# raulmur/ORB_SLAM2

Measured on NVIDIA H100. Metric: stereo frames/sec (ORB extract L+R + ComputeStereoMatches, KITTI-shaped 1242x375 @2000 kpts), higher is better.
Workload: dtype u8

## Files before the change

### include/borb.h

```cpp
#ifndef BORB_H
#define BORB_H

#include <stddef.h>
#include <stdint.h>

#if defined(__GNUC__)
#define BORB_API __attribute__((visibility("default")))
#else
#define BORB_API
#endif

#ifdef __cplusplus
extern "C" {
#endif

#define BORB_VERSION 2
#define BORB_MAX_LEVELS 16
#define BORB_MAX_DIM 4095

typedef enum borb_status {
    BORB_OK = 0,
    BORB_ERR_INVALID_ARG = 1,
    BORB_ERR_NO_DEVICE = 2,
    BORB_ERR_CUDA = 3,
    BORB_ERR_UNSUPPORTED = 4,
    BORB_ERR_CAPACITY = 5,
    BORB_ERR_STATE = 6
} borb_status;

typedef struct borb_keypoint {
    float x, y;
    float size;
    float angle;
    float response;
    int32_t octave;
    int32_t class_id;
} borb_keypoint;

typedef struct borb_extractor_cfg {
    int32_t n_features;
    float scale_factor;
    int32_t n_levels;
    int32_t ini_th_fast;
    int32_t min_th_fast;
} borb_extractor_cfg;

typedef struct borb_extractor borb_extractor;

BORB_API const char* borb_last_error(void);
BORB_API const char* borb_status_str(borb_status s);
BORB_API int borb_version(void);
BORB_API borb_status borb_device_count(int* n);

BORB_API borb_status borb_host_alloc(void** p, size_t bytes);
BORB_API borb_status borb_host_free(void* p);

BORB_API borb_status borb_extractor_create(const borb_extractor_cfg* cfg, int device, borb_extractor** out);
BORB_API borb_status borb_extractor_destroy(borb_extractor* e);
BORB_API borb_status borb_extractor_tables(const borb_extractor* e, float* scale, float* inv_scale, float* sigma2,
                                  float* inv_sigma2, int32_t* features_per_level);
BORB_API borb_status borb_extractor_capacity(const borb_extractor* e, int width, int height, int* cap);
BORB_API borb_status borb_extractor_reserve(borb_extractor* e, int width, int height, int max_images);

BORB_API borb_status borb_extract(borb_extractor* e, const uint8_t* gray, int width, int height, int stride,
                         borb_keypoint* kps, uint8_t* desc, int cap, int* n_out);

BORB_API borb_status borb_extract_batch(borb_extractor* e, const uint8_t* const* gray, int n_images, int width, int height,
                               int stride, borb_keypoint* kps, uint8_t* desc, int cap, int* n_out);

BORB_API borb_status borb_extract_batch_enqueue(borb_extractor* e, const uint8_t* const* gray, int n_images, int width,
                                       int height, int stride, borb_keypoint* kps, uint8_t* desc, int cap, int* n_out);
BORB_API borb_status borb_sync(borb_extractor* e);

BORB_API borb_status borb_extract_batch_device(borb_extractor* e, const uint8_t* d_gray, int n_images, int width, int height,
                                      size_t pitch, size_t image_stride, borb_keypoint* kps, uint8_t* desc, int cap,
                                      int* n_out);

BORB_API borb_status borb_extractor_set_input_format(borb_extractor* e, int channels, int rgb_order);

BORB_API borb_status borb_extractor_set_rectify_maps(borb_extractor* e, int which, const float* map_x, const float* map_y, int src_w,
                                                     int src_h, int dst_w, int dst_h);

BORB_API borb_status borb_extractor_pyramid(borb_extractor* e, int image, int level, uint8_t* dst, int* w, int* h);

BORB_API borb_status borb_stereo_match(borb_extractor* e, int n_pairs, const int* left_idx, const int* right_idx, float bf,
                              float b, float* u_right, float* depth, int cap);

BORB_API borb_status borb_stereo_match2(borb_extractor* left, borb_extractor* right, float bf, float b, float* u_right,
                               float* depth, int cap);

BORB_API borb_status borb_stereo_frames(borb_extractor* e, const uint8_t* const* left, const uint8_t* const* right, int n_pairs,
                               int width, int height, int stride, float bf, float b, borb_keypoint* kps_left,
                               uint8_t* desc_left, int* n_left, borb_keypoint* kps_right, uint8_t* desc_right,
                               int* n_right, float* u_right, float* depth, int cap);
BORB_API borb_status borb_stereo_frames_enqueue(borb_extractor* e, const uint8_t* const* left, const uint8_t* const* right,
                                       int n_pairs, int width, int height, int stride, float bf, float b,
                                       borb_keypoint* kps_left, uint8_t* desc_left, int* n_left,
                                       borb_keypoint* kps_right, uint8_t* desc_right, int* n_right, float* u_right,
                                       float* depth, int cap);
BORB_API borb_status borb_stereo_frames_device_enqueue(borb_extractor* e, const uint8_t* d_gray, int n_pairs, int width,
                                              int height, size_t pitch, size_t image_stride, float bf, float b,
                                              int* n_left, int* n_right, float* u_right, float* depth, int cap);
BORB_API borb_status borb_stereo_frames_device(borb_extractor* e, const uint8_t* d_gray, int n_pairs, int width, int height,
                                      size_t pitch, size_t image_stride, float bf, float b, int* n_left, int* n_right,
                                      float* u_right, float* depth, int cap);
BORB_API borb_status borb_stereo_frames_results(borb_extractor* e, int n_pairs, borb_keypoint* kps_left, uint8_t* desc_left,
                                                int* n_left, borb_keypoint* kps_right, uint8_t* desc_right, int* n_right,
                                                float* u_right, float* depth, int cap);

typedef struct borb_matcher borb_matcher;
#define BORB_MATCH_MAX_FEATURES 8192
BORB_API borb_status borb_matcher_create(int device, borb_matcher** out);
BORB_API borb_status borb_matcher_destroy(borb_matcher* m);

typedef struct borb_frame borb_frame;
typedef struct borb_frame_view {
    int32_t n;
    const borb_keypoint* keys_un;
    const uint8_t* desc;
    const float* u_right;
    const uint8_t* occupied;
    float min_x, min_y, max_x, max_y;
    int32_t n_levels;
    const float* scale_factors;
    const borb_frame* resident;
} borb_frame_view;

BORB_API borb_status borb_frame_create(borb_matcher* m, const borb_frame_view* view, borb_frame** out);
BORB_API borb_status borb_frame_destroy(borb_frame* f);

typedef struct borb_camera {
    float fx, fy, cx, cy;
    float k1, k2, p1, p2, k3;
    float bf;
} borb_camera;

BORB_API borb_status borb_frames_from_extractor(borb_matcher* m, borb_extractor* e, const int32_t* images, int n_frames,
                                                const int32_t* n_keys, const borb_camera* cam, int mode, const void* const* depth,
                                                int depth_type, float depth_factor, int depth_stride_bytes, borb_keypoint* keys_un,
                                                float* u_right, float* depth_out, int cap, float* bounds4, borb_frame** frames);
BORB_API borb_status borb_frame_info(const borb_frame* f, int32_t* n, int32_t* n_levels, int32_t* has_u_right);

typedef struct borb_mappoint_view {
    int32_t n;
    const float* proj_x;
    const float* proj_y;
    const float* proj_xr;
    const int32_t* level;
    const float* view_cos;
    const uint8_t* desc;
    const uint8_t* valid;
    const uint8_t* has_obs;
} borb_mappoint_view;

BORB_API borb_status borb_search_by_projection(borb_matcher* m, const borb_frame_view* frame, const borb_mappoint_view* mps,
                                               float th, float nnratio, int32_t* match_feat, int32_t* n_matches);
BORB_API borb_status borb_search_by_projection_batch(borb_matcher* m, const borb_frame_view* frames, const borb_mappoint_view* points,
                                                     int n_jobs, float th, float nnratio, int32_t* const* match_feat, int32_t* n_matches);

typedef struct borb_lastframe_view {
    int32_t n;
    const borb_keypoint* keys_un;
    const float* world_pos;
    const uint8_t* desc;
    const uint8_t* valid;
    const uint8_t* has_obs;
} borb_lastframe_view;

BORB_API borb_status borb_search_by_projection_last(borb_matcher* m, const borb_frame_view* cur, const borb_lastframe_view* last,
                                                    const float* Tcw, float fx, float fy, float cx, float cy, float bf, float th,
                                                    int forward, int backward, int check_orientation, int32_t* state_cur,
                                                    int32_t* n_matches);

typedef struct borb_worldpoints_view {
    int32_t n;
    const float* world_pos;
    const uint8_t* desc;
    const float* max_distance;
    const float* min_distance;
    const float* normal;
    const float* angle;
    const uint8_t* valid;
} borb_worldpoints_view;

BORB_API borb_status borb_search_by_projection_kf(borb_matcher* m, const borb_frame_view* cur, const borb_worldpoints_view* pts,
                                                  const float* Tcw, const float* Ow, float fx, float fy, float cx, float cy,
                                                  float log_scale_factor, float th, int orb_dist, int check_orientation,
                                                  int32_t* state_cur, int32_t* n_matches);

BORB_API borb_status borb_search_by_projection_sim3(borb_matcher* m, const borb_frame_view* kf, const borb_worldpoints_view* pts,
                                                    const float* Tcw, const float* Ow, float fx, float fy, float cx, float cy,
                                                    float log_scale_factor, int th, int32_t* state_kf, int32_t* n_matches);

BORB_API borb_status borb_fuse(borb_matcher* m, const borb_frame_view* kf, const float* inv_level_sigma2,
                               const borb_worldpoints_view* pts, const float* Tcw, const float* Ow, float fx, float fy, float cx,
                               float cy, float bf, float log_scale_factor, float th, int scw_variant, int32_t* best_idx,
                               int32_t* n_found);

BORB_API borb_status borb_search_by_sim3(borb_matcher* m, const borb_frame_view* kf1, const borb_frame_view* kf2,
                                         const borb_worldpoints_view* pts1, const borb_worldpoints_view* pts2, const float* T1w,
                                         const float* T2w, const float* S12, const float* S21, float fx, float fy, float cx, float cy,
                                         float log_scale_factor1, float log_scale_factor2, float th, int32_t* match12,
                                         int32_t* n_found);

BORB_API borb_status borb_search_local_points(borb_matcher* m, const borb_frame_view* frame, const borb_worldpoints_view* pts,
                                              const uint8_t* has_obs, const float* Tcw, const float* Ow, float fx, float fy, float cx,
                                              float cy, float mbf, float viewing_cos_limit, float log_scale_factor, float th,
                                              float nnratio, uint8_t* in_view, float* proj_x, float* proj_y, float* proj_xr,
                                              int32_t* level, float* view_cos, int32_t* match_feat, int32_t* n_matches);

typedef struct borb_local_points_job {
    borb_frame_view frame;
    borb_worldpoints_view pts;
    const uint8_t* has_obs;
    float Tcw[12];
    float Ow[3];
    float fx, fy, cx, cy, mbf;
    float log_scale_factor;
    float th;
    uint8_t* in_view;
    float* proj_x;
    float* proj_y;
    float* proj_xr;
    int32_t* level;
    float* view_cos;
    int32_t* match_feat;
} borb_local_points_job;
BORB_API borb_status borb_search_local_points_batch(borb_matcher* m, const borb_local_points_job* jobs, int n_jobs, float viewing_cos_limit,
                                                    float nnratio, int32_t* n_matches);

typedef struct borb_last_frame_job {
    borb_frame_view cur;
    borb_lastframe_view last;
    float Tcw[12];
    float fx, fy, cx, cy, bf;
    float th;
    int32_t forward, backward;
    int32_t* state_cur;
} borb_last_frame_job;
BORB_API borb_status borb_search_by_projection_last_batch(borb_matcher* m, const borb_last_frame_job* jobs, int n_jobs, int check_orientation,
                                                          int32_t* n_matches);

BORB_API borb_status borb_search_for_initialization(borb_matcher* m, const borb_frame_view* f1, const borb_frame_view* f2,
                                                    float* prev_matched, int window_size, float nnratio, int check_orientation,
                                                    int32_t* matches12, int32_t* n_matches);

BORB_API borb_status borb_distinctive_descriptors(borb_matcher* m, const uint8_t* desc, const int32_t* offsets, int n_points,
                                                  int32_t* best_idx);

typedef struct borb_featvec_view {
    int32_t n_nodes;
    const uint32_t* node_id;
    const int32_t* start;
    const uint32_t* feat_idx;
} borb_featvec_view;

typedef struct borb_keyframe_view {
    int32_t n;
    const borb_keypoint* keys_un;
    const uint8_t* desc;
    const uint8_t* has_mp;
    const float* u_right;
    borb_featvec_view fv;
    int32_t n_levels;
    const float* scale_factors;
    const float* level_sigma2;
} borb_keyframe_view;

BORB_API borb_status borb_search_by_bow(borb_matcher* m, const borb_keyframe_view* kfs, int n_kf, const borb_keyframe_view* frame,
                                        float nnratio, int check_orientation, int32_t* match, int32_t* n_matches);
BORB_API borb_status borb_search_by_bow_kf(borb_matcher* m, const borb_keyframe_view* kf1, const borb_keyframe_view* kf2,
                                           float nnratio, int check_orientation, int32_t* match12, int32_t* n_matches);

typedef struct borb_bow_job {
    const borb_frame* frame;
    borb_keyframe_view kf;
    const borb_frame* kf_frame;
    int32_t* match;
} borb_bow_job;
BORB_API borb_status borb_search_by_bow_batch(borb_matcher* m, const borb_bow_job* jobs, int n_jobs, float nnratio,
                                              int check_orientation, int32_t* n_matches);
BORB_API borb_status borb_search_for_triangulation(borb_matcher* m, const borb_keyframe_view* kf1, const borb_keyframe_view* kf2,
                                                   const float* F12, float ex, float ey, int only_stereo, int check_orientation,
                                                   int32_t* pairs, int cap, int32_t* n_pairs);

typedef struct borb_kfdb borb_kfdb;
BORB_API borb_status borb_kfdb_create(int device, borb_kfdb** out);
BORB_API borb_status borb_kfdb_destroy(borb_kfdb* db);
BORB_API borb_status borb_kfdb_clear(borb_kfdb* db);
BORB_API borb_status borb_kfdb_add(borb_kfdb* db, const borb_keyframe_view* kf, const uint32_t* bow_word, const double* bow_value,
                                   int n_bow, int32_t* slot_out);
BORB_API borb_status borb_kfdb_erase(borb_kfdb* db, int32_t slot);
BORB_API borb_status borb_kfdb_set_has_mp(borb_kfdb* db, int32_t slot, const uint8_t* has_mp);
BORB_API borb_status borb_kfdb_size(const borb_kfdb* db, int32_t* n_slots, uint64_t* device_bytes);
BORB_API borb_status borb_kfdb_query(borb_matcher* m, borb_kfdb* db, const uint32_t* bow_word, const double* bow_value, int n_bow,
                                     int32_t* common_words, float* score, uint32_t* first_word, int cap, int32_t* n_slots);
BORB_API borb_status borb_search_by_bow_db(borb_matcher* m, borb_kfdb* db, const int32_t* slots, int n_kf,
                                           const borb_keyframe_view* frame, float nnratio, int check_orientation, int32_t* match,
                                           int32_t* n_matches);

BORB_API borb_status borb_search_by_bow_db_pairs(borb_matcher* m, borb_kfdb* db, const int32_t* slots, int n_kf,
                                                 const borb_keyframe_view* frame, float nnratio, int check_orientation,
                                                 int32_t* n_matches, int32_t* pair_offset, uint32_t* pairs, int pairs_cap,
                                                 int32_t* n_pairs_total);

typedef struct borb_voc borb_voc;
BORB_API borb_status borb_voc_create(const int32_t* parent, const uint8_t* is_leaf, const uint8_t* desc, const double* weight,
                                     int n_nodes, int k, int L, int device, borb_voc** out);
BORB_API borb_status borb_voc_load_text(const char* path, int device, borb_voc** out);
BORB_API borb_status borb_voc_destroy(borb_voc* v);
BORB_API borb_status borb_voc_blob(const borb_voc* v, void** d_blob, size_t* bytes);
BORB_API borb_status borb_voc_from_blob(void* d_blob, size_t bytes, int device, borb_voc** out);
BORB_API borb_status borb_nccl_unique_id(uint8_t* id128);
BORB_API borb_status borb_nccl_comm_create(const uint8_t* id128, int world_size, int rank, int device, void** nccl_comm);
BORB_API borb_status borb_nccl_comm_destroy(void* nccl_comm);
BORB_API borb_status borb_voc_broadcast(borb_voc* root_voc, void* nccl_comm, int root, int rank, int device, borb_voc** out);

BORB_API borb_status borb_bow_transform(borb_voc* v, const uint8_t* desc, int n, int levelsup, int32_t* word, double* weight,
                                        int32_t* node);

BORB_API borb_status borb_compute_bow(borb_voc* v, const uint8_t* desc, int n, int levelsup, uint32_t* bow_word, double* bow_value,
                                      int32_t* n_bow, uint32_t* fv_node, int32_t* fv_start, uint32_t* fv_idx, int32_t* n_nodes);

BORB_API borb_status borb_frames_compute_bow(borb_matcher* m, borb_voc* v, borb_frame* const* frames, int n_frames, int levelsup,
                                             uint32_t* const* bow_word, double* const* bow_value, int32_t* n_bow,
                                             uint32_t* const* fv_node, int32_t* const* fv_start, uint32_t* const* fv_idx,
                                             int32_t* n_nodes);

BORB_API borb_status borb_matcher_set_timing(borb_matcher* m, int enable);
BORB_API borb_status borb_matcher_last_kernel_ms(borb_matcher* m, float* ms);
BORB_API borb_status borb_matcher_launch_count(const borb_matcher* m, uint64_t* n);
BORB_API borb_status borb_debug_candidates(borb_extractor* e, int image, int level, int32_t* xys, int cap, int* n_out);
BORB_API borb_status borb_debug_selected(borb_extractor* e, int image, int level, int32_t* xys, int cap, int* n_out);
BORB_API borb_status borb_debug_blurred(borb_extractor* e, int image, int level, uint8_t* dst, int* w, int* h);
BORB_API borb_status borb_debug_set_fast_mode(borb_extractor* e, int mode);
BORB_API borb_status borb_debug_brief_slots(uint32_t* dst, int cap, int* n_bins);
BORB_API borb_status borb_debug_set_bow_csa(int mode);
BORB_API borb_status borb_debug_set_bow_item_target(int target);
BORB_API borb_status borb_launch_count(const borb_extractor* e, uint64_t* n);
BORB_API borb_status borb_stage_times(borb_extractor* e, float* ms8);
BORB_API borb_status borb_set_timing(borb_extractor* e, int enable);
BORB_API borb_status borb_stage_times_total(borb_extractor* e, double* ms8, uint64_t* steps);
BORB_API borb_status borb_extractor_stream(borb_extractor* e, void** stream);

#ifdef __cplusplus
}
#endif
#endif
```

### orb_slam2_b200/_lib.py

```python
from __future__ import annotations

import ctypes as C
import os

import numpy as np

HERE = os.path.dirname(os.path.abspath(__file__))
LIB_PATH = os.path.join(HERE, "libborb.so")

KP_DTYPE = np.dtype([("x", "<f4"), ("y", "<f4"), ("size", "<f4"), ("angle", "<f4"), ("response", "<f4"),
                     ("octave", "<i4"), ("class_id", "<i4")])

BORB_OK = 0
STATUS_NAMES = {0: "BORB_OK", 1: "BORB_ERR_INVALID_ARG", 2: "BORB_ERR_NO_DEVICE", 3: "BORB_ERR_CUDA",
                4: "BORB_ERR_UNSUPPORTED", 5: "BORB_ERR_CAPACITY", 6: "BORB_ERR_STATE"}


class BorbError(RuntimeError):
    def __init__(self, status: int, where: str, detail: str):
        self.status = status
        super().__init__(f"{where}: {STATUS_NAMES.get(status, status)}: {detail}")


class ExtractorCfg(C.Structure):
    _fields_ = [("n_features", C.c_int32), ("scale_factor", C.c_float), ("n_levels", C.c_int32),
                ("ini_th_fast", C.c_int32), ("min_th_fast", C.c_int32)]


u8p = C.POINTER(C.c_uint8)
f32p = C.POINTER(C.c_float)
i32p = C.POINTER(C.c_int32)
vp = C.c_void_p

_SIGNATURES = {
    "borb_last_error": (C.c_char_p, []),
    "borb_status_str": (C.c_char_p, [C.c_int]),
    "borb_version": (C.c_int, []),
    "borb_device_count": (C.c_int, [i32p]),
    "borb_host_alloc": (C.c_int, [C.POINTER(vp), C.c_size_t]),
    "borb_host_free": (C.c_int, [vp]),
    "borb_extractor_create": (C.c_int, [C.POINTER(ExtractorCfg), C.c_int, C.POINTER(vp)]),
    "borb_extractor_destroy": (C.c_int, [vp]),
    "borb_extractor_tables": (C.c_int, [vp, f32p, f32p, f32p, f32p, i32p]),
    "borb_extractor_capacity": (C.c_int, [vp, C.c_int, C.c_int, i32p]),
    "borb_extractor_reserve": (C.c_int, [vp, C.c_int, C.c_int, C.c_int]),
    "borb_extract": (C.c_int, [vp, vp, C.c_int, C.c_int, C.c_int, vp, vp, C.c_int, i32p]),
    "borb_extract_batch": (C.c_int, [vp, C.POINTER(vp), C.c_int, C.c_int, C.c_int, C.c_int, vp, vp, C.c_int, vp]),
    "borb_extract_batch_enqueue": (C.c_int, [vp, C.POINTER(vp), C.c_int, C.c_int, C.c_int, C.c_int, vp, vp, C.c_int, vp]),
    "borb_sync": (C.c_int, [vp]),
    "borb_extract_batch_device": (C.c_int, [vp, vp, C.c_int, C.c_int, C.c_int, C.c_size_t, C.c_size_t, vp, vp, C.c_int, vp]),
    "borb_extractor_pyramid": (C.c_int, [vp, C.c_int, C.c_int, vp, i32p, i32p]),
    "borb_stereo_match": (C.c_int, [vp, C.c_int, vp, vp, C.c_float, C.c_float, vp, vp, C.c_int]),
    "borb_stereo_match2": (C.c_int, [vp, vp, C.c_float, C.c_float, vp, vp, C.c_int]),
    "borb_stereo_frames": (C.c_int, [vp, C.POINTER(vp), C.POINTER(vp), C.c_int, C.c_int, C.c_int, C.c_int, C.c_float,
                                     C.c_float, vp, vp, vp, vp, vp, vp, vp, vp, C.c_int]),
    "borb_stereo_frames_enqueue": (C.c_int, [vp, C.POINTER(vp), C.POINTER(vp), C.c_int, C.c_int, C.c_int, C.c_int,
                                             C.c_float, C.c_float, vp, vp, vp, vp, vp, vp, vp, vp, C.c_int]),
    "borb_stereo_frames_device": (C.c_int, [vp, vp, C.c_int, C.c_int, C.c_int, C.c_size_t, C.c_size_t, C.c_float,
                                            C.c_float, vp, vp, vp, vp, C.c_int]),
    "borb_stereo_frames_device_enqueue": (C.c_int, [vp, vp, C.c_int, C.c_int, C.c_int, C.c_size_t, C.c_size_t, C.c_float,
                                                    C.c_float, vp, vp, vp, vp, C.c_int]),
    "borb_stereo_frames_results": (C.c_int, [vp, C.c_int, vp, vp, vp, vp, vp, vp, vp, vp, C.c_int]),
    "borb_stage_times_total": (C.c_int, [vp, C.POINTER(C.c_double), C.POINTER(C.c_uint64)]),
    "borb_extractor_stream": (C.c_int, [vp, C.POINTER(vp)]),
    "borb_matcher_create": (C.c_int, [C.c_int, C.POINTER(vp)]),
    "borb_extractor_set_input_format": (C.c_int, [vp, C.c_int, C.c_int]),
    "borb_extractor_set_rectify_maps": (C.c_int, [vp, C.c_int, vp, vp, C.c_int, C.c_int, C.c_int, C.c_int]),
    "borb_matcher_destroy": (C.c_int, [vp]),
    "borb_frame_create": (C.c_int, [vp, vp, C.POINTER(vp)]),
    "borb_frame_destroy": (C.c_int, [vp]),
    "borb_frames_from_extractor": (C.c_int, [vp, vp, vp, C.c_int, vp, vp, C.c_int, vp, C.c_int, C.c_float, C.c_int, vp, vp, vp, C.c_int, vp, vp]),
    "borb_frame_info": (C.c_int, [vp, i32p, i32p, i32p]),
    "borb_search_by_projection": (C.c_int, [vp, vp, vp, C.c_float, C.c_float, vp, i32p]),
    "borb_search_by_projection_batch": (C.c_int, [vp, vp, vp, C.c_int, C.c_float, C.c_float, vp, vp]),
    "borb_search_by_projection_last": (C.c_int, [vp, vp, vp, vp, C.c_float, C.c_float, C.c_float, C.c_float, C.c_float, C.c_float,
                                                 C.c_int, C.c_int, C.c_int, vp, i32p]),
    "borb_search_by_projection_kf": (C.c_int, [vp, vp, vp, vp, vp, C.c_float, C.c_float, C.c_float, C.c_float, C.c_float, C.c_float,
                                               C.c_int, C.c_int, vp, i32p]),
    "borb_search_by_projection_sim3": (C.c_int, [vp, vp, vp, vp, vp, C.c_float, C.c_float, C.c_float, C.c_float, C.c_float, C.c_int,
                                                 vp, i32p]),
    "borb_search_for_initialization": (C.c_int, [vp, vp, vp, vp, C.c_int, C.c_float, C.c_int, vp, i32p]),
    "borb_distinctive_descriptors": (C.c_int, [vp, vp, vp, C.c_int, vp]),
    "borb_kfdb_create": (C.c_int, [C.c_int, C.POINTER(vp)]),
    "borb_kfdb_destroy": (C.c_int, [vp]),
    "borb_kfdb_clear": (C.c_int, [vp]),
    "borb_kfdb_add": (C.c_int, [vp, vp, vp, vp, C.c_int, i32p]),
    "borb_kfdb_erase": (C.c_int, [vp, C.c_int32]),
    "borb_kfdb_set_has_mp": (C.c_int, [vp, C.c_int32, vp]),
    "borb_kfdb_size": (C.c_int, [vp, i32p, C.POINTER(C.c_uint64)]),
    "borb_kfdb_query": (C.c_int, [vp, vp, vp, vp, C.c_int, vp, vp, vp, C.c_int, i32p]),
    "borb_search_by_bow_db": (C.c_int, [vp, vp, vp, C.c_int, vp, C.c_float, C.c_int, vp, vp]),
    "borb_search_by_bow_db_pairs": (C.c_int, [vp, vp, vp, C.c_int, vp, C.c_float, C.c_int, vp, vp, vp, C.c_int, i32p]),
    "borb_search_local_points": (C.c_int, [vp, vp, vp, vp, vp, vp] + [C.c_float] * 9 + [vp] * 7 + [i32p]),
    "borb_search_local_points_batch": (C.c_int, [vp, vp, C.c_int, C.c_float, C.c_float, vp]),
    "borb_search_by_projection_last_batch": (C.c_int, [vp, vp, C.c_int, C.c_int, vp]),
    "borb_fuse": (C.c_int, [vp, vp, vp, vp, vp, vp, C.c_float, C.c_float, C.c_float, C.c_float, C.c_float, C.c_float, C.c_float, C.c_int,
                            vp, i32p]),
    "borb_search_by_sim3": (C.c_int, [vp, vp, vp, vp, vp, vp, vp, vp, vp, C.c_float, C.c_float, C.c_float, C.c_float, C.c_float, C.c_float,
                                      C.c_float, vp, i32p]),
    "borb_search_by_bow": (C.c_int, [vp, vp, C.c_int, vp, C.c_float, C.c_int, vp, vp]),
    "borb_search_by_bow_kf": (C.c_int, [vp, vp, vp, C.c_float, C.c_int, vp, i32p]),
    "borb_search_by_bow_batch": (C.c_int, [vp, vp, C.c_int, C.c_float, C.c_int, vp]),
    "borb_frames_compute_bow": (C.c_int, [vp, vp, vp, C.c_int, C.c_int, vp, vp, vp, vp, vp, vp, vp]),
    "borb_search_for_triangulation": (C.c_int, [vp, vp, vp, vp, C.c_float, C.c_float, C.c_int, C.c_int, vp, C.c_int, i32p]),
    "borb_voc_create": (C.c_int, [vp, vp, vp, vp, C.c_int, C.c_int, C.c_int, C.c_int, C.POINTER(vp)]),
    "borb_voc_load_text": (C.c_int, [C.c_char_p, C.c_int, C.POINTER(vp)]),
    "borb_voc_destroy": (C.c_int, [vp]),
    "borb_voc_blob": (C.c_int, [vp, C.POINTER(vp), C.POINTER(C.c_size_t)]),
    "borb_voc_from_blob": (C.c_int, [vp, C.c_size_t, C.c_int, C.POINTER(vp)]),
    "borb_bow_transform": (C.c_int, [vp, vp, C.c_int, C.c_int, vp, vp, vp]),
    "borb_debug_candidates": (C.c_int, [vp, C.c_int, C.c_int, vp, C.c_int, i32p]),
    "borb_debug_selected": (C.c_int, [vp, C.c_int, C.c_int, vp, C.c_int, i32p]),
    "borb_debug_blurred": (C.c_int, [vp, C.c_int, C.c_int, vp, i32p, i32p]),
    "borb_nccl_unique_id": (C.c_int, [vp]),
    "borb_nccl_comm_create": (C.c_int, [vp, C.c_int, C.c_int, C.c_int, C.POINTER(vp)]),
    "borb_nccl_comm_destroy": (C.c_int, [vp]),
    "borb_voc_broadcast": (C.c_int, [vp, vp, C.c_int, C.c_int, C.c_int, C.POINTER(vp)]),
    "borb_compute_bow": (C.c_int, [vp, vp, C.c_int, C.c_int, vp, vp, i32p, vp, vp, vp, i32p]),
    "borb_matcher_set_timing": (C.c_int, [vp, C.c_int]),
    "borb_matcher_last_kernel_ms": (C.c_int, [vp, f32p]),
    "borb_matcher_launch_count": (C.c_int, [vp, C.POINTER(C.c_uint64)]),
    "borb_debug_set_bow_csa": (C.c_int, [C.c_int]),
    "borb_debug_set_bow_item_target": (C.c_int, [C.c_int]),
    "borb_debug_set_fast_mode": (C.c_int, [vp, C.c_int]),
    "borb_debug_brief_slots": (C.c_int, [vp, C.c_int, i32p]),
    "borb_launch_count": (C.c_int, [vp, C.POINTER(C.c_uint64)]),
    "borb_stage_times": (C.c_int, [vp, f32p]),
    "borb_set_timing": (C.c_int, [vp, C.c_int]),
}

_lib = None


def exported_names():
    return sorted(_SIGNATURES)


def load() -> C.CDLL:
    global _lib
    if _lib is not None:
        return _lib
    if not os.path.exists(LIB_PATH):
        raise ImportError(f"{LIB_PATH} is missing: build it with `python -c 'import __graft_entry__ as g; g.build()'` "
                          "(orb_slam2_b200 has no CPU fallback)")
    lib = C.CDLL(LIB_PATH)
    for name, (res, args) in _SIGNATURES.items():
        fn = getattr(lib, name)
        fn.restype = res
        fn.argtypes = args
    _lib = lib
    return lib


def check(status: int, where: str) -> None:
    if status != BORB_OK:
        detail = load().borb_last_error()
        raise BorbError(status, where, detail.decode() if detail else "")


def device_count() -> int:
    n = C.c_int32(0)
    st = load().borb_device_count(C.byref(n))
    return n.value if st == BORB_OK else 0


def ptr(a: np.ndarray):
    return a.ctypes.data_as(vp) if a is not None else None
```

### orb_slam2_b200/csrc/borb_host.cu

```cuda
#include <cmath>
#include <cstdarg>
#include <cstdio>
#include <algorithm>
#include <cstdlib>
#include <cstring>

#include "borb_internal.h"

namespace borb {

static thread_local std::string tl_error;
void set_error(const char* fmt, ...) {
    char buf[512];
    va_list ap;
    va_start(ap, fmt);
    vsnprintf(buf, sizeof(buf), fmt, ap);
    va_end(ap);
    tl_error = buf;
}

bool allow_max_smem(const void* func) {
    static std::mutex mu;
    static std::vector<std::pair<const void*, int>> done;
    int dev = 0;
    if (cudaGetDevice(&dev) != cudaSuccess) return false;
    std::lock_guard<std::mutex> lk(mu);
    for (auto& d : done)
        if (d.first == func && d.second == dev) return true;
    cudaFuncAttributes fa;
    int optin = 0;
    cudaError_t e = cudaFuncGetAttributes(&fa, func);
    if (e == cudaSuccess) e = cudaDeviceGetAttribute(&optin, cudaDevAttrMaxSharedMemoryPerBlockOptin, dev);
    if (e == cudaSuccess) e = cudaFuncSetAttribute(func, cudaFuncAttributeMaxDynamicSharedMemorySize, optin - (int)fa.sharedSizeBytes);
    if (e != cudaSuccess) { set_error("raising the shared-memory limit failed: %s", cudaGetErrorString(e)); cudaGetLastError(); return false; }
    done.push_back({func, dev});
    return true;
}

namespace {

inline int cv_round_f(float v) { return (int)lrintf(v); }
inline int align_up(int v, int a) { return (v + a - 1) / a * a; }

void init_tables(borb_extractor* e) {
    const int L = e->cfg.n_levels;
    const double sf = (double)e->cfg.scale_factor;
    e->scale.assign(L, 1.f); e->sigma2.assign(L, 1.f); e->inv_scale.assign(L, 1.f); e->inv_sigma2.assign(L, 1.f);
    for (int i = 1; i < L; i++) {
        e->scale[i] = (float)((double)e->scale[i - 1] * sf);
        e->sigma2[i] = e->scale[i] * e->scale[i];
    }
    for (int i = 0; i < L; i++) { e->inv_scale[i] = 1.0f / e->scale[i]; e->inv_sigma2[i] = 1.0f / e->sigma2[i]; }
    e->per_level.assign(L, 0);
    const float factor = (float)(1.0 / sf);
    float want = (float)e->cfg.n_features * (1.f - factor) / (1.f - (float)std::pow((double)factor, (double)L));
    int sum = 0;
    for (int l = 0; l < L - 1; l++) {
        e->per_level[l] = cv_round_f(want);
        sum += e->per_level[l];
        want *= factor;
    }
    e->per_level[L - 1] = e->cfg.n_features - sum > 0 ? e->cfg.n_features - sum : 0;
    const int vmax = (int)std::floor(HALF_PATCH * std::sqrt(2.f) / 2 + 1);
    const int vmin = (int)std::ceil(HALF_PATCH * std::sqrt(2.f) / 2);
    for (int v = 0; v < 16; v++) e->umax[v] = 0;
    for (int v = 0; v <= vmax; ++v) e->umax[v] = (int)lrint(std::sqrt((double)HALF_PATCH * HALF_PATCH - (double)v * v));
    for (int v = HALF_PATCH, v0 = 0; v >= vmin; --v) {
        while (e->umax[v0] == e->umax[v0 + 1]) ++v0;
        e->umax[v] = v0;
        ++v0;
    }
}

void resize_table(int src, int dst, bool clamp_edges, int extra, std::vector<int16_t>& out) {
    const double inv = (double)dst / src, scale = 1. / inv;
    const size_t first = out.size();
    for (int d = 0; d < dst; d++) {
        float f = (float)((d + 0.5) * scale - 0.5);
        int s = (int)std::floor(f);
        f -= s;
        if (clamp_edges) {
            if (s < 0) { f = 0; s = 0; }
            if (s >= src - 1) { f = 0; s = src - 1; }
        }
        out.push_back((int16_t)s);
        out.push_back((int16_t)cv_round_f((1.f - f) * 2048.f));
        out.push_back((int16_t)cv_round_f(f * 2048.f));
        out.push_back(0);
    }
    for (int k = 0; k < extra; k++) {
        int r = 2 * dst - 2 - (dst + k);
        if (r < 0) r = 0;
        for (int j = 0; j < 4; j++) out.push_back(out[first + (size_t)r * 4 + j]);
    }
    if (((out.size() - first) / 4) & 1) for (int j = 0; j < 4; j++) out.push_back(0);
}

bool resize_window_table(const std::vector<int16_t>& tabs, size_t xtab_first, int n_entries, std::vector<int16_t>& out) {
    bool ok = true;
    for (int gq = 0; gq < n_entries; gq += 4) {
        int lo = 1 << 30, hi = 0;
        for (int i = 0; i < 4; i++) {
            const int ofs = tabs[xtab_first + (size_t)(gq + i) * 4];
            lo = std::min(lo, ofs); hi = std::max(hi, ofs);
        }
        const int base = lo & ~3;
        if (hi + 1 - base > 11) ok = false;
        for (int i = 0; i < 4; i++) {
            const int16_t* e = &tabs[xtab_first + (size_t)(gq + i) * 4];
            const int pos = e[0] - base;
            int s1 = 0, s2 = 0x10;
            if (pos <= 6) s1 = pos | ((pos + 1) << 4);
            else if (pos == 7) { s1 = 7; s2 = 0x40; }
            else { const int q = (pos - 8) + 4; s2 = q | ((q + 1) << 4); }
            out.push_back(e[1]);
            out.push_back(e[2]);
            out.push_back((int16_t)base);
            out.push_back((int16_t)((s1 | (s2 << 8)) & 0x7FFF));
        }
    }
    return ok;
}

const int8_t kPattern[1024] = {
#include "orb_pattern.inc"
};

borb_status build_geometry(borb_extractor* e, int w, int h, std::vector<int16_t>& tabs) {
    Geometry& g = e->geom;
    std::memset(&g, 0, sizeof(g));
    const int L = e->cfg.n_levels;
    g.nlevels = L; g.w = w; g.h = h;
    g.fast_mode = e->fast_mode;
    g.ini_th = e->cfg.ini_th_fast < 0 ? 0 : (e->cfg.ini_th_fast > 255 ? 255 : e->cfg.ini_th_fast);
    g.min_th = e->cfg.min_th_fast < 0 ? 0 : (e->cfg.min_th_fast > 255 ? 255 : e->cfg.min_th_fast);
    for (int i = 0; i < 16; i++) g.umax[i] = e->umax[i];
    unsigned pyr_off = 0, cand_off = 0;
    int blk = 0, sel_off = 0, btile = 0;
    tabs.clear();
    for (int l = 0; l < L; l++) {
        LevelGeom& v = g.lv[l];
        v.w = cv_round_f((float)w * e->inv_scale[l]);
        v.h = cv_round_f((float)h * e->inv_scale[l]);
        const float width = (float)(v.w - 2 * MIN_BORDER), height = (float)(v.h - 2 * MIN_BORDER);
        v.nCols = (int)(width / 30.f);
        v.nRows = (int)(height / 30.f);
        if (v.nCols < 1 || v.nRows < 1) {
            set_error("level %d is %dx%d: too small for the 30-px FAST cell grid (reference divides by zero)", l, v.w, v.h);
            return BORB_ERR_UNSUPPORTED;
        }
        v.wCell = (int)std::ceil(width / v.nCols);
        v.hCell = (int)std::ceil(height / v.nRows);
        v.pitch = align_up(v.w + 8, 128);
        v.pyr_off = pyr_off;
        pyr_off += (unsigned)v.pitch * v.h;
        v.cellsPerBlk = FAST_TILE_W / v.wCell > 0 ? FAST_TILE_W / v.wCell : 1;
        v.rowsPerBlk = fast_rows_per_blk(v.nRows, v.hCell);
        v.blkCols = (v.nCols + v.cellsPerBlk - 1) / v.cellsPerBlk;
        v.blkBase = blk;
        blk += v.blkCols * ((v.nRows + v.rowsPerBlk - 1) / v.rowsPerBlk);
        v.cand_off = cand_off;
        v.cand_cap = v.nCols * v.nRows * ((v.wCell + 1) / 2) * ((v.hCell + 1) / 2);
        cand_off += (unsigned)align_up(v.cand_cap, 32);
        v.quota = e->per_level[l];
        v.nIni = (int)std::round(width / height);
        if (v.nIni < 1) { set_error("level %d aspect ratio gives zero quadtree roots (reference divides by zero)", l); return BORB_ERR_UNSUPPORTED; }
        v.hX = width / v.nIni;
        v.node_cap = (v.quota > 4 * v.nIni ? v.quota : 4 * v.nIni) + 3;
        v.node_cap = align_up(v.node_cap + 1, 4);
        v.sel_off = sel_off;
        sel_off += v.node_cap;
        v.scale = e->scale[l];
        v.inv_scale = e->inv_scale[l];
        v.patch_size = (float)(int)(PATCH * e->scale[l]);
        g.blur_base[l] = btile;
        btile += ((v.w + BLUR_TILE_W - 1) / BLUR_TILE_W) * ((v.h + BLUR_TILE_H - 1) / BLUR_TILE_H);
        if (l > 0) {
            const int wpad = (v.w + 8 + 3) & ~3;
            v.xtab_off = (unsigned)(tabs.size() / 4);
            resize_table(g.lv[l - 1].w, v.w, true, wpad - v.w, tabs);
            v.ytab_off = (unsigned)(tabs.size() / 4);
            resize_table(g.lv[l - 1].h, v.h, false, 0, tabs);
            v.xwin_off = (unsigned)(tabs.size() / 4);
            std::vector<int16_t> win;
            v.x_windowed = resize_window_table(tabs, (size_t)v.xtab_off * 4, wpad, win) ? 1 : 0;
            tabs.insert(tabs.end(), win.begin(), win.end());
        }
        if (quadtree_smem_bytes(v.node_cap) > 200 * 1024) {
            set_error("per-level quota %d exceeds the quadtree kernel's shared-memory envelope", v.quota);
            return BORB_ERR_UNSUPPORTED;
        }
    }
    g.blur_base[L] = btile;
    g.blur_tiles = btile;
    g.fast_blocks = blk;
    g.pyr_image_stride = (unsigned)align_up((int)pyr_off, g.lv[0].pitch);
    g.cand_image_stride = cand_off;
    g.sel_image_stride = sel_off;
    if (sel_off >= 65536) { set_error("keypoint capacity %d exceeds 65535", sel_off); return BORB_ERR_UNSUPPORTED; }
    return BORB_OK;
}

void free_workspace(Workspace& ws) {
    cudaFree(ws.pyr); cudaFree(ws.blur); cudaFree(ws.cand); cudaFree(ws.cand_cnt); cudaFree(ws.pnode); cudaFree(ws.sel);
    cudaFree(ws.sel_cnt); cudaFree(ws.kps); cudaFree(ws.desc); cudaFree(ws.nkp); cudaFree(ws.u_right); cudaFree(ws.depth);
    cudaFree(ws.sad); cudaFree(ws.tabs); cudaFree(ws.brief_slots); cudaFree(ws.pair_idx); cudaFree(ws.st_bins); cudaFree(ws.st_recs); cudaFree(ws.stage);
    free(ws.fast_tmaps); cudaFree(ws.fast_tiles);
    ws = Workspace();
}

borb_status ensure(borb_extractor* e, int w, int h, int n_images) {
    if (w < 1 || h < 1 || w > BORB_MAX_DIM || h > BORB_MAX_DIM) { set_error("image size %dx%d outside [1,%d]", w, h, BORB_MAX_DIM); return BORB_ERR_UNSUPPORTED; }
    BORB_CUDA(cudaSetDevice(e->device));
    const bool same_shape = e->have_geom && e->geom.w == w && e->geom.h == h;
    if (same_shape && e->ws.max_images >= n_images) return BORB_OK;
    BORB_CUDA(cudaStreamSynchronize(e->stream));
    std::vector<int16_t> tabs;
    e->have_geom = false;
    e->last_n_images = 0;
    e->last_stereo_pairs = 0;
    borb_status st = build_geometry(e, w, h, tabs);
    if (st != BORB_OK) return st;
    size_t n = (size_t)(n_images > 2 ? n_images : 2);
    if (same_shape && (size_t)e->ws.max_images > n) n = (size_t)e->ws.max_images;
    free_workspace(e->ws);
    if (e->h_counts) { cudaFreeHost(e->h_counts); e->h_counts = nullptr; }
    e->pair_cache.clear();
    const Geometry& g = e->geom;
    Workspace& ws = e->ws;
    BORB_CUDA(cudaMalloc(&ws.pyr, n * g.pyr_image_stride + 256));
    BORB_CUDA(cudaMalloc(&ws.blur, n * g.pyr_image_stride + 256));
    BORB_CUDA(cudaMalloc(&ws.cand, n * g.cand_image_stride * sizeof(uint32_t)));
    BORB_CUDA(cudaMalloc(&ws.pnode, n * g.cand_image_stride * sizeof(int)));
    BORB_CUDA(cudaMalloc(&ws.cand_cnt, n * g.nlevels * sizeof(int)));
    BORB_CUDA(cudaMalloc(&ws.sel, n * g.sel_image_stride * sizeof(uint32_t)));
    BORB_CUDA(cudaMalloc(&ws.sel_cnt, n * g.nlevels * sizeof(int)));
    BORB_CUDA(cudaMalloc(&ws.kps, n * g.sel_image_stride * sizeof(borb_keypoint)));
    BORB_CUDA(cudaMalloc(&ws.desc, n * g.sel_image_stride * 32));
    BORB_CUDA(cudaMalloc(&ws.nkp, n * sizeof(int)));
    BORB_CUDA(cudaMalloc(&ws.u_right, n * g.sel_image_stride * sizeof(float)));
    BORB_CUDA(cudaMalloc(&ws.depth, n * g.sel_image_stride * sizeof(float)));
    BORB_CUDA(cudaMalloc(&ws.sad, n * g.sel_image_stride * sizeof(int)));
    BORB_CUDA(cudaMalloc(&ws.pair_idx, n * 2 * sizeof(int)));
    BORB_CUDA(cudaMalloc(&ws.st_bins, n * stereo_bins_bytes_per_pair()));
    BORB_CUDA(cudaMalloc(&ws.st_recs, n * (size_t)stereo_rec_stride(g) * stereo_rec_bytes()));
    BORB_CUDA(cudaMalloc(&ws.tabs, (tabs.size() + 4) * sizeof(int16_t)));
    BORB_CUDA(cudaMemcpy(ws.tabs, tabs.data(), tabs.size() * sizeof(int16_t), cudaMemcpyHostToDevice));
    const std::vector<uint32_t>& slots = brief_slot_table();
    BORB_CUDA(cudaMalloc(&ws.brief_slots, slots.size() * sizeof(uint32_t)));
    BORB_CUDA(cudaMemcpy(ws.brief_slots, slots.data(), slots.size() * sizeof(uint32_t), cudaMemcpyHostToDevice));
    BORB_CUDA(cudaMemset(ws.nkp, 0, n * sizeof(int)));
    BORB_CUDA(cudaMallocHost(&e->h_counts, n * 2 * sizeof(int)));
    ws.max_images = (int)n;
    ws.fast_tmaps = malloc(fast_tmaps_bytes());
    if ((st = build_fast_tmaps(g, ws, ws.fast_tmaps)) != BORB_OK) return st;
    if ((st = build_fast_tiles(g, ws)) != BORB_OK) return st;
    e->have_geom = true;
    return BORB_OK;
}

void drain_timing(borb_extractor* e);
void begin_step(borb_extractor* e) {
    if (!e->timing) return;
    if (e->ev.empty()) {
        e->ev.resize((size_t)borb_extractor::EV_RING * 9);
        for (auto& x : e->ev) cudaEventCreate(&x);
    }
    if (e->ev_pending >= borb_extractor::EV_RING) {
        cudaStreamSynchronize(e->stream);
        drain_timing(e);
    }
    e->ev_slot = (e->ev_slot + 1) % borb_extractor::EV_RING;
    e->ev_mask[e->ev_slot] = 0;
    e->ev_pending++;
}
void mark(borb_extractor* e, int i) {
    if (!e->timing || e->ev.empty()) return;
    cudaEventRecord(e->ev[(size_t)e->ev_slot * 9 + i], e->stream);
    e->ev_mask[e->ev_slot] |= 1u << i;
}
void drain_timing(borb_extractor* e) {
    const int R = borb_extractor::EV_RING;
    for (int k = e->ev_pending - 1; k >= 0; k--) {
        const int slot = ((e->ev_slot - k) % R + R) % R;
        const unsigned m = e->ev_mask[slot];
        for (int i = 0; i < 8; i++) {
            float ms = 0.f;
            if (m & (1u << i)) {
                int j = i + 1;
                while (j < 9 && !(m & (1u << j))) j++;
                if (j < 9 && cudaEventElapsedTime(&ms, e->ev[(size_t)slot * 9 + i], e->ev[(size_t)slot * 9 + j]) != cudaSuccess) { ms = 0.f; cudaGetLastError(); }
            }
            e->stage_ms[i] = ms;
            e->stage_sum_ms[i] += ms;
        }
        e->stage_steps++;
    }
    e->ev_pending = 0;
}

borb_status enqueue_extract(borb_extractor* e, int n) {
    const Geometry& g = e->geom;
    Workspace& ws = e->ws;
    cudaStream_t s = e->stream;
    BORB_CUDA(cudaMemsetAsync(ws.cand_cnt, 0, (size_t)n * g.nlevels * sizeof(int), s));
    mark(e, 1);
    e->launches += launch_pyramid(g, ws, n, s);
    mark(e, 2);
    e->launches += launch_fast(g, ws, n, s);
    mark(e, 3);
    e->launches += launch_quadtree(g, ws, n, s);
    mark(e, 4);
    e->launches += launch_blur(g, ws, n, s);
    mark(e, 5);
    e->launches += launch_describe(g, ws, n, s);
    mark(e, 6);
    BORB_CUDA(cudaGetLastError());
    e->last_n_images = n;
    e->last_stereo_pairs = 0;
    return BORB_OK;
}

borb_status rectified_size(borb_extractor* e, int w, int h, int* gw, int* gh) {
    if (!e->d_map[0][0]) return BORB_OK;
    if (w != e->map_src_w || h != e->map_src_h) {
        set_error("rectification maps were built for %dx%d raw frames, got %dx%d", e->map_src_w, e->map_src_h, w, h);
        return BORB_ERR_INVALID_ARG;
    }
    *gw = e->map_dst_w; *gh = e->map_dst_h;
    return BORB_OK;
}

borb_status upload_slots(borb_extractor* e, const uint8_t* const* slots, int n, int w, int h, int stride, bool stereo_pairs = false) {
    const Geometry& g = e->geom;
    const int ch = e->in_channels;
    if (stride < w * ch) { set_error("stride %d smaller than a row of %d %d-channel pixels", stride, w, ch); return BORB_ERR_INVALID_ARG; }
    const size_t img_bytes = (size_t)stride * h;
    bool contiguous = n > 1 || ch > 1 || e->d_map[0][0] != nullptr;
    for (int k = 0; k < n; k++) {
        if (!slots[k]) { set_error("image %d is NULL", k); return BORB_ERR_INVALID_ARG; }
        if (slots[k] != slots[0] + (size_t)k * img_bytes) contiguous = false;
    }
    auto need_stage = [&](size_t need) -> borb_status {
        if (e->ws.stage_bytes < need) {
            BORB_CUDA(cudaStreamSynchronize(e->stream));
            cudaFree(e->ws.stage);
            e->ws.stage = nullptr; e->ws.stage_bytes = 0;
            BORB_CUDA(cudaMalloc(&e->ws.stage, need));
            e->ws.stage_bytes = need;
        }
        return BORB_OK;
    };
    if (e->d_map[0][0]) {
        if (ch != 1) { set_error("rectification maps apply to CV_8UC1 frames"); return BORB_ERR_UNSUPPORTED; }
        const size_t src_img = contiguous ? img_bytes : (size_t)w * h;
        const int src_stride = contiguous ? stride : w;
        borb_status st = need_stage(src_img * n);
        if (st != BORB_OK) return st;
        if (contiguous) BORB_CUDA(cudaMemcpyAsync(e->ws.stage, slots[0], src_img * n, cudaMemcpyHostToDevice, e->stream));
        else
            for (int k = 0; k < n; k++)
                BORB_CUDA(cudaMemcpy2DAsync(e->ws.stage + (size_t)k * src_img, w, slots[k], stride, w, h, cudaMemcpyHostToDevice, e->stream));
        e->launches += launch_repack_remap(g, e->ws, e->ws.stage, src_stride, src_img, w, h, e->d_map[0][0], e->d_map[0][1],
                                           stereo_pairs ? e->d_map[1][0] : nullptr, stereo_pairs ? e->d_map[1][1] : nullptr, n, e->stream);
        return BORB_OK;
    }
    if (contiguous) {
        const size_t need = img_bytes * n;
        borb_status st = need_stage(need);
        if (st != BORB_OK) return st;
        BORB_CUDA(cudaMemcpyAsync(e->ws.stage, slots[0], need, cudaMemcpyHostToDevice, e->stream));
        if (ch == 1) e->launches += launch_repack(g, e->ws, e->ws.stage, stride, img_bytes, n, e->stream);
        else e->launches += launch_repack_color(g, e->ws, e->ws.stage, stride, img_bytes, ch, e->in_rgb, n, e->stream);
        return BORB_OK;
    }
    if (ch > 1) {
        const size_t row = (size_t)w * ch;
        borb_status st = need_stage(row * h * n);
        if (st != BORB_OK) return st;
        for (int k = 0; k < n; k++)
            BORB_CUDA(cudaMemcpy2DAsync(e->ws.stage + (size_t)k * row * h, row, slots[k], stride, row, h, cudaMemcpyHostToDevice, e->stream));
        e->launches += launch_repack_color(g, e->ws, e->ws.stage, (int)row, row * h, ch, e->in_rgb, n, e->stream);
        return BORB_OK;
    }
    for (int k = 0; k < n; k++) {
        uint8_t* dst = e->ws.pyr + (size_t)k * g.pyr_image_stride + g.lv[0].pyr_off;
        BORB_CUDA(cudaMemcpy2DAsync(dst, g.lv[0].pitch, slots[k], stride, w, h, cudaMemcpyHostToDevice, e->stream));
    }
    return BORB_OK;
}

borb_status upload_device(borb_extractor* e, const uint8_t* d_gray, int n, int w, int h, size_t pitch, size_t image_stride) {
    const Geometry& g = e->geom;
    cudaMemcpy3DParms p = {};
    p.srcPtr = make_cudaPitchedPtr((void*)d_gray, pitch, w, image_stride / pitch);
    p.dstPtr = make_cudaPitchedPtr(e->ws.pyr + g.lv[0].pyr_off, g.lv[0].pitch, w, g.pyr_image_stride / g.lv[0].pitch);
    if (image_stride % pitch == 0 && g.pyr_image_stride % g.lv[0].pitch == 0) {
        p.extent = make_cudaExtent(w, h, n);
        p.kind = cudaMemcpyDeviceToDevice;
        BORB_CUDA(cudaMemcpy3DAsync(&p, e->stream));
    } else {
        for (int i = 0; i < n; i++)
            BORB_CUDA(cudaMemcpy2DAsync(e->ws.pyr + (size_t)i * g.pyr_image_stride + g.lv[0].pyr_off, g.lv[0].pitch,
                                        d_gray + (size_t)i * image_stride, pitch, w, h, cudaMemcpyDeviceToDevice, e->stream));
    }
    return BORB_OK;
}

borb_status download_kps(borb_extractor* e, int first, int count, int step, borb_keypoint* kps, uint8_t* desc, int cap, int* n_out) {
    const Geometry& g = e->geom;
    const int m = cap < g.sel_image_stride ? cap : g.sel_image_stride;
    cudaStream_t s = e->stream;
    if (kps && m > 0)
        BORB_CUDA(cudaMemcpy2DAsync(kps, (size_t)cap * sizeof(borb_keypoint), e->ws.kps + (size_t)first * g.sel_image_stride,
                                    (size_t)step * g.sel_image_stride * sizeof(borb_keypoint), (size_t)m * sizeof(borb_keypoint),
                                    count, cudaMemcpyDeviceToHost, s));
    if (desc && m > 0)
        BORB_CUDA(cudaMemcpy2DAsync(desc, (size_t)cap * 32, e->ws.desc + (size_t)first * g.sel_image_stride * 32,
                                    (size_t)step * g.sel_image_stride * 32, (size_t)m * 32, count, cudaMemcpyDeviceToHost, s));
    if (n_out)
        BORB_CUDA(cudaMemcpy2DAsync(n_out, sizeof(int), e->ws.nkp + first, (size_t)step * sizeof(int), sizeof(int), count,
                                    cudaMemcpyDeviceToHost, s));
    return BORB_OK;
}

borb_status check_args(borb_extractor* e, int n, int w, int h) {
    if (!e) { set_error("null handle"); return BORB_ERR_INVALID_ARG; }
    if (n < 0) { set_error("negative image count"); return BORB_ERR_INVALID_ARG; }
    (void)w; (void)h;
    return BORB_OK;
}

borb_status enqueue_stereo(borb_extractor* eL, borb_extractor* eR, int n_pairs, const int* left_idx, const int* right_idx,
                           float bf, float b) {
    borb_extractor* e = eL;
    const Geometry& g = e->geom;
    std::vector<int> idx(2 * (size_t)n_pairs);
    for (int p = 0; p < n_pairs; p++) {
        idx[2 * p] = left_idx ? left_idx[p] : (eL == eR ? 2 * p : 0);
        idx[2 * p + 1] = right_idx ? right_idx[p] : (eL == eR ? 2 * p + 1 : 0);
        if (idx[2 * p] < 0 || idx[2 * p] >= eL->last_n_images || idx[2 * p + 1] < 0 || idx[2 * p + 1] >= eR->last_n_images) {
            set_error("stereo pair %d refers to an image outside the last batch", p);
            return BORB_ERR_STATE;
        }
    }
    if (n_pairs > e->ws.max_images) { set_error("too many pairs"); return BORB_ERR_INVALID_ARG; }
    if (idx != e->pair_cache) {
        BORB_CUDA(cudaStreamSynchronize(e->stream));
        std::memcpy(e->h_counts, idx.data(), idx.size() * sizeof(int));
        BORB_CUDA(cudaMemcpyAsync(e->ws.pair_idx, e->h_counts, idx.size() * sizeof(int), cudaMemcpyHostToDevice, e->stream));
        e->pair_cache = idx;
    }
    StereoView L{eL->ws.pyr, eL->ws.kps, eL->ws.desc, eL->ws.nkp, eL->geom.pyr_image_stride, eL->geom.sel_image_stride};
    StereoView R{eR->ws.pyr, eR->ws.kps, eR->ws.desc, eR->ws.nkp, eR->geom.pyr_image_stride, eR->geom.sel_image_stride};
    mark(e, 6);
    e->launches += launch_stereo(g, L, R, e->ws.pair_idx, n_pairs, bf, b, e->ws.u_right, e->ws.depth, e->ws.sad, g.sel_image_stride, e->ws.st_bins, e->ws.st_recs, e->stream);
    mark(e, 7);
    BORB_CUDA(cudaGetLastError());
    e->last_stereo_pairs = (eL == eR && !left_idx && !right_idx) ? n_pairs : 0;
    return BORB_OK;
}

borb_status download_stereo(borb_extractor* e, int n_pairs, float* u_right, float* depth, int cap) {
    const Geometry& g = e->geom;
    const int m = cap < g.sel_image_stride ? cap : g.sel_image_stride;
    if (u_right && m > 0)
        BORB_CUDA(cudaMemcpy2DAsync(u_right, (size_t)cap * 4, e->ws.u_right, (size_t)g.sel_image_stride * 4, (size_t)m * 4, n_pairs, cudaMemcpyDeviceToHost, e->stream));
    if (depth && m > 0)
        BORB_CUDA(cudaMemcpy2DAsync(depth, (size_t)cap * 4, e->ws.depth, (size_t)g.sel_image_stride * 4, (size_t)m * 4, n_pairs, cudaMemcpyDeviceToHost, e->stream));
    return BORB_OK;
}

borb_status finish_timing(borb_extractor* e) {
    if (e->timing && e->ev_pending > 0) drain_timing(e);
    return BORB_OK;
}

}

const std::vector<uint32_t>& brief_slot_table() {
    static const std::vector<uint32_t> table = [] {
        std::vector<uint32_t> t((size_t)BRIEF_BINS * 512);
        int row[512], col[512], order[512];
        for (int b = 0; b < BRIEF_BINS; b++) {
            const double th = (b + 0.5) * (2.0 * 3.14159265358979323846 / BRIEF_BINS);
            const double a = std::cos(th), s = std::sin(th);
            for (int p = 0; p < 512; p++) {
                const int x = kPattern[2 * p], y = kPattern[2 * p + 1];
                row[p] = (int)std::lround(x * s + y * a);
                col[p] = (int)std::lround(x * a - y * s);
                order[p] = p;
            }
            std::sort(order, order + 512, [&](int i, int j) {
                return row[i] != row[j] ? row[i] < row[j] : (col[i] != col[j] ? col[i] < col[j] : i < j);
            });
            for (int k = 0; k < 512; k++) {
                const int p = order[k];
                t[(size_t)b * 512 + k] = (uint32_t)(kPattern[2 * p] + 128) | (uint32_t)(kPattern[2 * p + 1] + 128) << 8 | (uint32_t)p << 16;
            }
        }
        return t;
    }();
    return table;
}

}

using namespace borb;

extern "C" {

const char* borb_last_error(void) { return tl_error.c_str(); }
const char* borb_status_str(borb_status s) {
    switch (s) {
        case BORB_OK: return "ok";
        case BORB_ERR_INVALID_ARG: return "invalid argument";
        case BORB_ERR_NO_DEVICE: return "no CUDA device (libborb has no CPU path)";
        case BORB_ERR_CUDA: return "CUDA error";
        case BORB_ERR_UNSUPPORTED: return "unsupported shape or quota";
        case BORB_ERR_CAPACITY: return "output capacity too small";
        case BORB_ERR_STATE: return "invalid call order";
    }
    return "unknown";
}
int borb_version(void) { return BORB_VERSION; }

borb_status borb_device_count(int* n) {
    if (!n) return BORB_ERR_INVALID_ARG;
    *n = 0;
    cudaError_t err = cudaGetDeviceCount(n);
    if (err != cudaSuccess) { *n = 0; cudaGetLastError(); set_error("cudaGetDeviceCount: %s", cudaGetErrorString(err)); return BORB_ERR_NO_DEVICE; }
    return BORB_OK;
}

borb_status borb_host_alloc(void** p, size_t bytes) {
    if (!p) return BORB_ERR_INVALID_ARG;
    BORB_CUDA(cudaMallocHost(p, bytes));
    return BORB_OK;
}
borb_status borb_host_free(void* p) {
    if (p) BORB_CUDA(cudaFreeHost(p));
    return BORB_OK;
}

borb_status borb_extractor_create(const borb_extractor_cfg* cfg, int device, borb_extractor** out) {
    if (!cfg || !out) { set_error("null argument"); return BORB_ERR_INVALID_ARG; }
    *out = nullptr;
    if (cfg->n_levels < 1 || cfg->n_levels > BORB_MAX_LEVELS || cfg->n_features < 1 || !(cfg->scale_factor > 1.0f)) {
        set_error("bad extractor cfg (n_features=%d scale=%f levels=%d)", cfg->n_features, cfg->scale_factor, cfg->n_levels);
        return BORB_ERR_INVALID_ARG;
    }
    int ndev = 0;
    borb_status st = borb_device_count(&ndev);
    if (st != BORB_OK) return st;
    if (ndev < 1) { set_error("no CUDA device visible; libborb has no CPU fallback"); return BORB_ERR_NO_DEVICE; }
    if (device < 0 || device >= ndev) { set_error("device %d out of range (%d visible)", device, ndev); return BORB_ERR_INVALID_ARG; }
    borb_extractor* e = new borb_extractor();
    e->cfg = *cfg;
    e->device = device;
    init_tables(e);
    cudaError_t err = cudaSetDevice(device);
    if (err == cudaSuccess) err = cudaStreamCreateWithFlags(&e->stream, cudaStreamNonBlocking);
    if (err != cudaSuccess) {
        set_error("CUDA init failed: %s", cudaGetErrorString(err));
        delete e;
        return BORB_ERR_CUDA;
    }
    *out = e;
    return BORB_OK;
}

borb_status borb_extractor_destroy(borb_extractor* e) {
    if (!e) return BORB_OK;
    cudaSetDevice(e->device);
    if (e->stream) cudaStreamSynchronize(e->stream);
    free_workspace(e->ws);
    for (int a = 0; a < 2; a++)
        for (int c = 0; c < 2; c++) cudaFree(e->d_map[a][c]);
    if (e->h_counts) cudaFreeHost(e->h_counts);
    for (auto& x : e->ev) cudaEventDestroy(x);
    if (e->stream) cudaStreamDestroy(e->stream);
    delete e;
    return BORB_OK;
}

borb_status borb_extractor_tables(const borb_extractor* e, float* scale, float* inv_scale, float* sigma2, float* inv_sigma2,
                                  int32_t* features_per_level) {
    if (!e) return BORB_ERR_INVALID_ARG;
    for (int l = 0; l < e->cfg.n_levels; l++) {
        if (scale) scale[l] = e->scale[l];
        if (inv_scale) inv_scale[l] = e->inv_scale[l];
        if (sigma2) sigma2[l] = e->sigma2[l];
        if (inv_sigma2) inv_sigma2[l] = e->inv_sigma2[l];
        if (features_per_level) features_per_level[l] = e->per_level[l];
    }
    return BORB_OK;
}

borb_status borb_extractor_capacity(const borb_extractor* e, int width, int height, int* cap) {
    if (!e || !cap) return BORB_ERR_INVALID_ARG;
    borb_extractor tmp;
    tmp.cfg = e->cfg; tmp.scale = e->scale; tmp.inv_scale = e->inv_scale; tmp.per_level = e->per_level;
    std::memcpy(tmp.umax, e->umax, sizeof(tmp.umax));
    std::vector<int16_t> tabs;
    if (width < 1 || height < 1 || width > BORB_MAX_DIM || height > BORB_MAX_DIM) { set_error("image size out of range"); return BORB_ERR_UNSUPPORTED; }
    borb_status st = build_geometry(&tmp, width, height, tabs);
    if (st != BORB_OK) return st;
    *cap = tmp.geom.sel_image_stride;
    return BORB_OK;
}

borb_status borb_extractor_reserve(borb_extractor* e, int width, int height, int max_images) {
    if (!e || max_images < 1) return BORB_ERR_INVALID_ARG;
    return ensure(e, width, height, max_images);
}

borb_status borb_sync(borb_extractor* e) {
    if (!e) return BORB_ERR_INVALID_ARG;
    BORB_CUDA(cudaSetDevice(e->device));
    BORB_CUDA(cudaStreamSynchronize(e->stream));
    return finish_timing(e);
}

borb_status borb_extract_batch_enqueue(borb_extractor* e, const uint8_t* const* gray, int n, int w, int h, int stride,
                                       borb_keypoint* kps, uint8_t* desc, int cap, int* n_out) {
    borb_status st = check_args(e, n, w, h);
    if (st != BORB_OK) return st;
    if (n == 0) return BORB_OK;
    if (!gray || cap < 0 || stride < w) { set_error("bad arguments"); return BORB_ERR_INVALID_ARG; }
    int gw = w, gh = h;
    if ((st = rectified_size(e, w, h, &gw, &gh)) != BORB_OK) return st;
    if ((st = ensure(e, gw, gh, n)) != BORB_OK) return st;
    begin_step(e);
    mark(e, 0);
    if ((st = upload_slots(e, gray, n, w, h, stride)) != BORB_OK) return st;
    if ((st = enqueue_extract(e, n)) != BORB_OK) return st;
    mark(e, 7);
    st = download_kps(e, 0, n, 1, kps, desc, cap, n_out);
    mark(e, 8);
    return st;
}

borb_status borb_extract_batch(borb_extractor* e, const uint8_t* const* gray, int n, int w, int h, int stride,
                               borb_keypoint* kps, uint8_t* desc, int cap, int* n_out) {
    if (!n_out) { set_error("n_out is required"); return BORB_ERR_INVALID_ARG; }
    borb_status st = borb_extract_batch_enqueue(e, gray, n, w, h, stride, kps, desc, cap, n_out);
    if (st != BORB_OK) return st;
    if (n == 0) return BORB_OK;
    if ((st = borb_sync(e)) != BORB_OK) return st;
    for (int i = 0; i < n; i++)
        if (n_out[i] > cap) { set_error("image %d produced %d keypoints, capacity %d", i, n_out[i], cap); return BORB_ERR_CAPACITY; }
    return BORB_OK;
}

borb_status borb_extract(borb_extractor* e, const uint8_t* gray, int w, int h, int stride, borb_keypoint* kps, uint8_t* desc,
                         int cap, int* n_out) {
    if (!n_out) { set_error("n_out is required"); return BORB_ERR_INVALID_ARG; }
    *n_out = 0;
    if (!gray || w == 0 || h == 0) return BORB_OK;
    const uint8_t* one[1] = {gray};
    return borb_extract_batch(e, one, 1, w, h, stride, kps, desc, cap, n_out);
}

borb_status borb_extract_batch_device(borb_extractor* e, const uint8_t* d_gray, int n, int w, int h, size_t pitch,
                                      size_t image_stride, borb_keypoint* kps, uint8_t* desc, int cap, int* n_out) {
    borb_status st = check_args(e, n, w, h);
    if (st != BORB_OK) return st;
    if (n == 0) return BORB_OK;
    if (!d_gray || pitch < (size_t)w) { set_error("bad arguments"); return BORB_ERR_INVALID_ARG; }
    if ((st = ensure(e, w, h, n)) != BORB_OK) return st;
    begin_step(e);
    mark(e, 0);
    if ((st = upload_device(e, d_gray, n, w, h, pitch, image_stride)) != BORB_OK) return st;
    if ((st = enqueue_extract(e, n)) != BORB_OK) return st;
    mark(e, 7);
    if ((st = download_kps(e, 0, n, 1, kps, desc, cap, n_out)) != BORB_OK) return st;
    mark(e, 8);
    return borb_sync(e);
}

borb_status borb_extractor_set_rectify_maps(borb_extractor* e, int which, const float* map_x, const float* map_y, int src_w, int src_h,
                                            int dst_w, int dst_h) {
    if (!e || which < 0 || which > 1) { set_error("bad arguments"); return BORB_ERR_INVALID_ARG; }
    BORB_CUDA(cudaSetDevice(e->device));
    BORB_CUDA(cudaStreamSynchronize(e->stream));
    if (!map_x || !map_y) {
        for (int s2 = which; s2 < 2; s2++)
            for (int c = 0; c < 2; c++) { cudaFree(e->d_map[s2][c]); e->d_map[s2][c] = nullptr; }
        return BORB_OK;
    }
    if (src_w <= 0 || src_h <= 0 || dst_w <= 0 || dst_h <= 0) { set_error("bad map geometry"); return BORB_ERR_INVALID_ARG; }
    if (which == 1 && (!e->d_map[0][0] || src_w != e->map_src_w || src_h != e->map_src_h || dst_w != e->map_dst_w || dst_h != e->map_dst_h)) {
        set_error("install the left maps (set 0) first; both sets share one geometry"); return BORB_ERR_STATE;
    }
    const size_t bytes = (size_t)dst_w * dst_h * sizeof(float);
    const float* src[2] = {map_x, map_y};
    for (int c = 0; c < 2; c++) {
        cudaFree(e->d_map[which][c]); e->d_map[which][c] = nullptr;
        BORB_CUDA(cudaMalloc(&e->d_map[which][c], bytes));
        BORB_CUDA(cudaMemcpy(e->d_map[which][c], src[c], bytes, cudaMemcpyHostToDevice));
    }
    if (which == 0) {
        e->map_src_w = src_w; e->map_src_h = src_h; e->map_dst_w = dst_w; e->map_dst_h = dst_h;
        for (int c = 0; c < 2; c++) { cudaFree(e->d_map[1][c]); e->d_map[1][c] = nullptr; }
    }
    return BORB_OK;
}

borb_status borb_extractor_set_input_format(borb_extractor* e, int channels, int rgb_order) {
    if (!e) { set_error("null handle"); return BORB_ERR_INVALID_ARG; }
    if (channels != 1 && channels != 3 && channels != 4) { set_error("channels must be 1, 3 or 4 (CV_8UC1 / C3 / C4)"); return BORB_ERR_INVALID_ARG; }
    e->in_channels = channels;
    e->in_rgb = rgb_order ? 1 : 0;
    return BORB_OK;
}

borb_status borb_extractor_pyramid(borb_extractor* e, int image, int level, uint8_t* dst, int* w, int* h) {
    if (!e || !e->have_geom || image < 0 || image >= e->last_n_images || level < 0 || level >= e->geom.nlevels) {
        set_error("no such image/level in the last batch");
        return BORB_ERR_STATE;
    }
    const LevelGeom& L = e->geom.lv[level];
    if (w) *w = L.w;
    if (h) *h = L.h;
    if (!dst) return BORB_OK;
    BORB_CUDA(cudaSetDevice(e->device));
    BORB_CUDA(cudaMemcpy2DAsync(dst, L.w, e->ws.pyr + (size_t)image * e->geom.pyr_image_stride + L.pyr_off, L.pitch, L.w, L.h,
                                cudaMemcpyDeviceToHost, e->stream));
    BORB_CUDA(cudaStreamSynchronize(e->stream));
    return BORB_OK;
}

borb_status borb_debug_blurred(borb_extractor* e, int image, int level, uint8_t* dst, int* w, int* h) {
    if (!e || !e->have_geom || image < 0 || image >= e->last_n_images || level < 0 || level >= e->geom.nlevels) {
        set_error("no such image/level in the last batch");
        return BORB_ERR_STATE;
    }
    const LevelGeom& L = e->geom.lv[level];
    if (w) *w = L.w;
    if (h) *h = L.h;
    if (!dst) return BORB_OK;
    BORB_CUDA(cudaSetDevice(e->device));
    BORB_CUDA(cudaMemcpy2DAsync(dst, L.w, e->ws.blur + (size_t)image * e->geom.pyr_image_stride + L.pyr_off, L.pitch, L.w, L.h,
                                cudaMemcpyDeviceToHost, e->stream));
    BORB_CUDA(cudaStreamSynchronize(e->stream));
    return BORB_OK;
}

static borb_status debug_list(borb_extractor* e, int image, int level, bool selected, int32_t* xys, int cap, int* n_out) {
    if (!e || !n_out || !e->have_geom || image < 0 || image >= e->last_n_images || level < 0 || level >= e->geom.nlevels) {
        set_error("no such image/level in the last batch");
        return BORB_ERR_STATE;
    }
    const Geometry& g = e->geom;
    const LevelGeom& L = g.lv[level];
    BORB_CUDA(cudaSetDevice(e->device));
    BORB_CUDA(cudaStreamSynchronize(e->stream));
    int n = 0;
    BORB_CUDA(cudaMemcpy(&n, (selected ? e->ws.sel_cnt : e->ws.cand_cnt) + image * g.nlevels + level, sizeof(int), cudaMemcpyDeviceToHost));
    *n_out = n;
    const int m = n < cap ? n : cap;
    if (m <= 0 || !xys) return BORB_OK;
    std::vector<uint32_t> raw(m);
    const uint32_t* src = selected ? e->ws.sel + (size_t)image * g.sel_image_stride + L.sel_off
                                   : e->ws.cand + (size_t)image * g.cand_image_stride + L.cand_off;
    BORB_CUDA(cudaMemcpy(raw.data(), src, (size_t)m * sizeof(uint32_t), cudaMemcpyDeviceToHost));
    for (int i = 0; i < m; i++) { xys[3 * i] = xys_x(raw[i]); xys[3 * i + 1] = xys_y(raw[i]); xys[3 * i + 2] = xys_s(raw[i]); }
    return BORB_OK;
}
borb_status borb_debug_candidates(borb_extractor* e, int image, int level, int32_t* xys, int cap, int* n_out) {
    return debug_list(e, image, level, false, xys, cap, n_out);
}
borb_status borb_debug_selected(borb_extractor* e, int image, int level, int32_t* xys, int cap, int* n_out) {
    return debug_list(e, image, level, true, xys, cap, n_out);
}

borb_status borb_debug_set_fast_mode(borb_extractor* e, int mode) {
    if (!e || mode < 0 || mode > 3) { set_error("fast mode must be 0..3"); return BORB_ERR_INVALID_ARG; }
    e->fast_mode = mode;
    if (e->have_geom) e->geom.fast_mode = mode;
    return BORB_OK;
}

borb_status borb_debug_brief_slots(uint32_t* dst, int cap, int* n_bins) {
    if (!n_bins) { set_error("n_bins is NULL"); return BORB_ERR_INVALID_ARG; }
    const std::vector<uint32_t>& t = brief_slot_table();
    *n_bins = BRIEF_BINS;
    if (dst) std::memcpy(dst, t.data(), std::min((size_t)(cap > 0 ? cap : 0), t.size()) * sizeof(uint32_t));
    return BORB_OK;
}

borb_status borb_launch_count(const borb_extractor* e, uint64_t* n) {
    if (!e || !n) return BORB_ERR_INVALID_ARG;
    *n = e->launches;
    return BORB_OK;
}
borb_status borb_set_timing(borb_extractor* e, int enable) {
    if (!e) return BORB_ERR_INVALID_ARG;
    e->timing = enable != 0;
    for (int i = 0; i < 8; i++) { e->stage_sum_ms[i] = 0; e->stage_ms[i] = 0; }
    e->stage_steps = 0;
    e->ev_pending = 0;
    return BORB_OK;
}
borb_status borb_stage_times_total(borb_extractor* e, double* ms8, uint64_t* steps) {
    if (!e || !ms8 || !steps) return BORB_ERR_INVALID_ARG;
    for (int i = 0; i < 8; i++) ms8[i] = e->stage_sum_ms[i];
    *steps = e->stage_steps;
    return BORB_OK;
}
borb_status borb_extractor_stream(borb_extractor* e, void** stream) {
    if (!e || !stream) return BORB_ERR_INVALID_ARG;
    *stream = (void*)e->stream;
    return BORB_OK;
}
borb_status borb_stage_times(borb_extractor* e, float* ms8) {
    if (!e || !ms8) return BORB_ERR_INVALID_ARG;
    for (int i = 0; i < 8; i++) ms8[i] = e->stage_ms[i];
    return BORB_OK;
}

borb_status borb_stereo_match(borb_extractor* e, int n_pairs, const int* left_idx, const int* right_idx, float bf, float b,
                              float* u_right, float* depth, int cap) {
    if (!e || n_pairs < 0 || !(b > 0.f)) { set_error("bad arguments"); return BORB_ERR_INVALID_ARG; }
    if (!e->have_geom || e->last_n_images == 0) { set_error("stereo match before any extract"); return BORB_ERR_STATE; }
    if (n_pairs == 0) return BORB_OK;
    BORB_CUDA(cudaSetDevice(e->device));
    begin_step(e);
    borb_status st = enqueue_stereo(e, e, n_pairs, left_idx, right_idx, bf, b);
    if (st != BORB_OK) return st;
    if ((st = download_stereo(e, n_pairs, u_right, depth, cap)) != BORB_OK) return st;
    mark(e, 8);
    return borb_sync(e);
}

borb_status borb_stereo_match2(borb_extractor* left, borb_extractor* right, float bf, float b, float* u_right, float* depth, int cap) {
    if (!left || !right || !(b > 0.f)) { set_error("bad arguments"); return BORB_ERR_INVALID_ARG; }
    if (!left->have_geom || !right->have_geom || left->last_n_images < 1 || right->last_n_images < 1) { set_error("stereo match before extract"); return BORB_ERR_STATE; }
    if (left->device != right->device || left->geom.w != right->geom.w || left->geom.h != right->geom.h ||
        left->geom.nlevels != right->geom.nlevels) {
        set_error("left/right extractors differ in device or geometry");
        return BORB_ERR_INVALID_ARG;
    }
    BORB_CUDA(cudaSetDevice(left->device));
    BORB_CUDA(cudaStreamSynchronize(right->stream));
    begin_step(left);
    borb_status st = enqueue_stereo(left, right, 1, nullptr, nullptr, bf, b);
    if (st != BORB_OK) return st;
    if ((st = download_stereo(left, 1, u_right, depth, cap)) != BORB_OK) return st;
    mark(left, 8);
    return borb_sync(left);
}

borb_status borb_stereo_frames_enqueue(borb_extractor* e, const uint8_t* const* left, const uint8_t* const* right, int n_pairs,
                                       int w, int h, int stride, float bf, float b, borb_keypoint* kps_left, uint8_t* desc_left,
                                       int* n_left, borb_keypoint* kps_right, uint8_t* desc_right, int* n_right, float* u_right,
                                       float* depth, int cap) {
    borb_status st = check_args(e, n_pairs, w, h);
    if (st != BORB_OK) return st;
    if (n_pairs == 0) return BORB_OK;
    if (!left || !right || stride < w || !(b > 0.f)) { set_error("bad arguments"); return BORB_ERR_INVALID_ARG; }
    int gw = w, gh = h;
    if ((st = rectified_size(e, w, h, &gw, &gh)) != BORB_OK) return st;
    if ((st = ensure(e, gw, gh, 2 * n_pairs)) != BORB_OK) return st;
    begin_step(e);
    mark(e, 0);
    {
        std::vector<const uint8_t*> slots(2 * (size_t)n_pairs);
        for (int p = 0; p < n_pairs; p++) { slots[2 * p] = left[p]; slots[2 * p + 1] = right[p]; }
        if ((st = upload_slots(e, slots.data(), 2 * n_pairs, w, h, stride, true)) != BORB_OK) return st;
    }
    if ((st = enqueue_extract(e, 2 * n_pairs)) != BORB_OK) return st;
    if ((st = enqueue_stereo(e, e, n_pairs, nullptr, nullptr, bf, b)) != BORB_OK) return st;
    if ((st = download_kps(e, 0, n_pairs, 2, kps_left, desc_left, cap, n_left)) != BORB_OK) return st;
    if ((st = download_kps(e, 1, n_pairs, 2, kps_right, desc_right, cap, n_right)) != BORB_OK) return st;
    if ((st = download_stereo(e, n_pairs, u_right, depth, cap)) != BORB_OK) return st;
    mark(e, 8);
    return BORB_OK;
}

borb_status borb_stereo_frames(borb_extractor* e, const uint8_t* const* left, const uint8_t* const* right, int n_pairs, int w,
                               int h, int stride, float bf, float b, borb_keypoint* kps_left, uint8_t* desc_left, int* n_left,
                               borb_keypoint* kps_right, uint8_t* desc_right, int* n_right, float* u_right, float* depth, int cap) {
    borb_status st = borb_stereo_frames_enqueue(e, left, right, n_pairs, w, h, stride, bf, b, kps_left, desc_left, n_left,
                                                kps_right, desc_right, n_right, u_right, depth, cap);
    if (st != BORB_OK || n_pairs == 0) return st;
    if ((st = borb_sync(e)) != BORB_OK) return st;
    for (int p = 0; p < n_pairs; p++)
        if ((n_left && n_left[p] > cap) || (n_right && n_right[p] > cap)) { set_error("pair %d exceeds capacity %d", p, cap); return BORB_ERR_CAPACITY; }
    return BORB_OK;
}

borb_status borb_stereo_frames_device_enqueue(borb_extractor* e, const uint8_t* d_gray, int n_pairs, int w, int h, size_t pitch,
                                              size_t image_stride, float bf, float b, int* n_left, int* n_right, float* u_right,
                                              float* depth, int cap) {
    borb_status st = check_args(e, n_pairs, w, h);
    if (st != BORB_OK) return st;
    if (n_pairs == 0) return BORB_OK;
    if (!d_gray || pitch < (size_t)w || !(b > 0.f)) { set_error("bad arguments"); return BORB_ERR_INVALID_ARG; }
    if ((st = ensure(e, w, h, 2 * n_pairs)) != BORB_OK) return st;
    begin_step(e);
    mark(e, 0);
    if ((st = upload_device(e, d_gray, 2 * n_pairs, w, h, pitch, image_stride)) != BORB_OK) return st;
    if ((st = enqueue_extract(e, 2 * n_pairs)) != BORB_OK) return st;
    if ((st = enqueue_stereo(e, e, n_pairs, nullptr, nullptr, bf, b)) != BORB_OK) return st;
    if ((st = download_kps(e, 0, n_pairs, 2, nullptr, nullptr, cap, n_left)) != BORB_OK) return st;
    if ((st = download_kps(e, 1, n_pairs, 2, nullptr, nullptr, cap, n_right)) != BORB_OK) return st;
    if ((st = download_stereo(e, n_pairs, u_right, depth, cap)) != BORB_OK) return st;
    mark(e, 8);
    return BORB_OK;
}

borb_status borb_stereo_frames_device(borb_extractor* e, const uint8_t* d_gray, int n_pairs, int w, int h, size_t pitch,
                                      size_t image_stride, float bf, float b, int* n_left, int* n_right, float* u_right,
                                      float* depth, int cap) {
    borb_status st = borb_stereo_frames_device_enqueue(e, d_gray, n_pairs, w, h, pitch, image_stride, bf, b, n_left, n_right,
                                                       u_right, depth, cap);
    if (st != BORB_OK || n_pairs == 0) return st;
    return borb_sync(e);
}

borb_status borb_stereo_frames_results(borb_extractor* e, int n_pairs, borb_keypoint* kps_left, uint8_t* desc_left, int* n_left,
                                       borb_keypoint* kps_right, uint8_t* desc_right, int* n_right, float* u_right, float* depth,
                                       int cap) {
    if (!e || n_pairs < 0 || cap < 0) { set_error("bad arguments"); return BORB_ERR_INVALID_ARG; }
    if (n_pairs == 0) return BORB_OK;
    if (!e->have_geom || n_pairs > e->last_stereo_pairs) {
        set_error("the last call on this handle left stereo results for %d pairs, %d requested", e->last_stereo_pairs, n_pairs);
        return BORB_ERR_STATE;
    }
    BORB_CUDA(cudaSetDevice(e->device));
    borb_status st;
    if ((st = download_kps(e, 0, n_pairs, 2, kps_left, desc_left, cap, n_left)) != BORB_OK) return st;
    if ((st = download_kps(e, 1, n_pairs, 2, kps_right, desc_right, cap, n_right)) != BORB_OK) return st;
    if ((st = download_stereo(e, n_pairs, u_right, depth, cap)) != BORB_OK) return st;
    if ((st = borb_sync(e)) != BORB_OK) return st;
    std::vector<int> counts(2 * (size_t)n_pairs);
    BORB_CUDA(cudaMemcpy(counts.data(), e->ws.nkp, counts.size() * sizeof(int), cudaMemcpyDeviceToHost));
    for (size_t i = 0; i < counts.size(); i++)
        if (counts[i] > cap) { set_error("pair %d exceeds capacity %d", (int)(i / 2), cap); return BORB_ERR_CAPACITY; }
    return BORB_OK;
}

}
```

### orb_slam2_b200/csrc/borb_internal.h

```cpp
#pragma once
#include <cuda_runtime.h>
#include <stdint.h>

#include <mutex>
#include <string>
#include <vector>

#include "../../include/borb.h"

namespace borb {

constexpr int EDGE = 19;
constexpr int PATCH = 31;
constexpr int HALF_PATCH = 15;
constexpr int MIN_BORDER = 16;
constexpr int TH_HIGH = 100;
constexpr int TH_LOW = 50;
constexpr int BLUR_TILE_W = 120;
constexpr int BLUR_TILE_H = 64;
constexpr int FAST_TILE_W = 124;
constexpr int FAST_H_BAND = 64;

__host__ __device__ inline int fast_rows_per_blk(int nRows, int hCell) {
    const int r = FAST_H_BAND / hCell;
    return r < 1 ? 1 : (r > nRows ? nRows : r);
}
__host__ __device__ inline int fast_box_rows(int rowsPerBlk, int hCell) { return rowsPerBlk * hCell + 6; }

__host__ __device__ inline uint32_t pack_xys(int x, int y, int s) { return (uint32_t)x | ((uint32_t)y << 12) | ((uint32_t)s << 24); }
__host__ __device__ inline int xys_x(uint32_t v) { return (int)(v & 0xFFFu); }
__host__ __device__ inline int xys_y(uint32_t v) { return (int)((v >> 12) & 0xFFFu); }
__host__ __device__ inline int xys_s(uint32_t v) { return (int)(v >> 24); }

struct LevelGeom {
    int w, h;
    int pitch;
    unsigned pyr_off;
    int nCols, nRows, wCell, hCell;
    int cellsPerBlk;
    int rowsPerBlk;
    int blkCols;
    int blkBase;
    unsigned cand_off;
    int cand_cap;
    int quota;
    int nIni;
    float hX;
    int node_cap;
    int sel_off;
    float scale;
    float inv_scale;
    float patch_size;
    unsigned xtab_off, ytab_off;
    unsigned xwin_off;
    int x_windowed;
};

struct Geometry {
    int nlevels;
    int w, h;
    int ini_th, min_th;
    int fast_mode;
    int fast_blocks;
    unsigned pyr_image_stride;
    unsigned cand_image_stride;
    int sel_image_stride;
    int blur_tiles;
    int blur_base[BORB_MAX_LEVELS + 1];
    int umax[16];
    LevelGeom lv[BORB_MAX_LEVELS];
};

struct Workspace {
    int max_images = 0;
    uint8_t* pyr = nullptr;
    uint8_t* blur = nullptr;
    uint32_t* cand = nullptr;
    int* cand_cnt = nullptr;
    int* pnode = nullptr;
    uint32_t* sel = nullptr;
    int* sel_cnt = nullptr;
    borb_keypoint* kps = nullptr;
    uint8_t* desc = nullptr;
    int* nkp = nullptr;
    float* u_right = nullptr;
    float* depth = nullptr;
    int* sad = nullptr;
    int16_t* tabs = nullptr;
    uint32_t* brief_slots = nullptr;
    int* pair_idx = nullptr;
    int* st_bins = nullptr;
    void* st_recs = nullptr;
    uint8_t* stage = nullptr;
    size_t stage_bytes = 0;
    void* fast_tmaps = nullptr;
    void* fast_tiles = nullptr;
    int fast_n_tiles = 0;
};

constexpr int BRIEF_BINS = 32;
const std::vector<uint32_t>& brief_slot_table();

void set_error(const char* fmt, ...);
bool allow_max_smem(const void* func);
#define BORB_CUDA(call)                                                                             \
    do {                                                                                            \
        cudaError_t _e = (call);                                                                    \
        if (_e != cudaSuccess) {                                                                    \
            borb::set_error("%s failed: %s (%s:%d)", #call, cudaGetErrorString(_e), __FILE__, __LINE__); \
            return (_e == cudaErrorNoDevice || _e == cudaErrorInsufficientDriver) ? BORB_ERR_NO_DEVICE : BORB_ERR_CUDA; \
        }                                                                                           \
    } while (0)

int launch_repack_remap(const Geometry& g, const Workspace& ws, const uint8_t* stage, int src_stride, size_t src_image_bytes, int src_w,
                        int src_h, const float* mx0, const float* my0, const float* mx1, const float* my1, int n_images, cudaStream_t s);
int launch_repack_color(const Geometry& g, const Workspace& ws, const uint8_t* stage, int src_stride, size_t src_image_bytes, int channels,
                        int rgb, int n_images, cudaStream_t s);
int launch_repack(const Geometry& g, const Workspace& ws, const uint8_t* stage, int src_stride, size_t src_image_bytes,
                  int n_images, cudaStream_t s);
int launch_pyramid(const Geometry& g, const Workspace& ws, int n_images, cudaStream_t s);
int launch_fast(const Geometry& g, const Workspace& ws, int n_images, cudaStream_t s);
int launch_quadtree(const Geometry& g, const Workspace& ws, int n_images, cudaStream_t s);
int launch_blur(const Geometry& g, const Workspace& ws, int n_images, cudaStream_t s);
int launch_describe(const Geometry& g, const Workspace& ws, int n_images, cudaStream_t s);

struct StereoView {
    const uint8_t* pyr;
    const borb_keypoint* kps;
    const uint8_t* desc;
    const int* nkp;
    unsigned pyr_image_stride;
    int kp_image_stride;
};
int launch_stereo(const Geometry& g, const StereoView& L, const StereoView& R, const int* d_pair_idx, int n_pairs,
                  float bf, float b, float* d_u_right, float* d_depth, int* d_sad, int out_stride, int* d_bins, void* d_recs,
                  cudaStream_t s);
int stereo_rec_stride(const Geometry& g);
size_t stereo_bins_bytes_per_pair();
size_t stereo_rec_bytes();
size_t quadtree_smem_bytes(int node_cap);
borb_status build_fast_tmaps(const Geometry& g, const Workspace& ws, void* out_tmaps);
borb_status build_fast_tiles(const Geometry& g, Workspace& ws);
size_t fast_tmaps_bytes();

}

struct borb_extractor {
    borb_extractor_cfg cfg;
    int device = 0;
    cudaStream_t stream = nullptr;
    std::vector<float> scale, inv_scale, sigma2, inv_sigma2;
    std::vector<int> per_level;
    int umax[16];
    bool have_geom = false;
    borb::Geometry geom;
    borb::Workspace ws;
    int last_n_images = 0;
    int last_stereo_pairs = 0;
    int in_channels = 1;
    int in_rgb = 1;
    float* d_map[2][2] = {{nullptr, nullptr}, {nullptr, nullptr}};
    int map_src_w = 0, map_src_h = 0, map_dst_w = 0, map_dst_h = 0;
    int fast_mode = 0;
    uint64_t launches = 0;
    static constexpr int EV_RING = 128;
    bool timing = false;
    std::vector<cudaEvent_t> ev;
    unsigned ev_mask[EV_RING] = {};
    int ev_slot = 0;
    int ev_pending = 0;
    float stage_ms[8] = {};
    double stage_sum_ms[8] = {};
    uint64_t stage_steps = 0;
    int* h_counts = nullptr;
    std::vector<int> pair_cache;
};
```

### orb_slam2_b200/csrc/k_blur.cu

```cuda
#include "borb_internal.h"

namespace borb {

namespace {
constexpr int BT_R = 16;
constexpr int BT_WARPS = BLUR_TILE_H / BT_R;

__device__ __forceinline__ int reflect101(int p, int len) {
    if (p < 0) p = -p;
    if (p >= len) p = 2 * len - 2 - p;
    return min(max(p, 0), len - 1);
}
}

__global__ void __launch_bounds__(32 * BT_WARPS) blur_kernel(const __grid_constant__ Geometry g, const uint8_t* __restrict__ pyr,
                                                             uint8_t* __restrict__ blur) {
    const int img = blockIdx.y;
    int l = 0;
    while (l + 1 < g.nlevels && (int)blockIdx.x >= g.blur_base[l + 1]) l++;
    const LevelGeom& L = g.lv[l];
    const int local = blockIdx.x - g.blur_base[l];
    const int tilesX = (L.w + BLUR_TILE_W - 1) / BLUR_TILE_W;
    const int ty = local / tilesX, tx = local - ty * tilesX;
    const int lane = threadIdx.x & 31, wrp = threadIdx.x >> 5;
    const int x = tx * BLUR_TILE_W + 4 * (lane - 1);
    const int yb = ty * BLUR_TILE_H + wrp * BT_R;
    if (yb >= L.h) return;
    const uint8_t* src = pyr + (size_t)img * g.pyr_image_stride + L.pyr_off;
    uint8_t* dst = blur + (size_t)img * g.pyr_image_stride + L.pyr_off;
    const int W = L.w, H = L.h, pitch = L.pitch;
    const bool left_edge = (x == 0);
    const bool loads = x >= 0 && x < pitch;
    const bool stores = lane >= 1 && lane <= 30 && x < W;
    const unsigned WLO = 18u | (34u << 8) | (48u << 16) | (56u << 24);
    const unsigned WHI = 48u | (34u << 8) | (18u << 16);

    uint32_t own[BT_R + 6];
    if (yb >= 3 && yb + BT_R + 2 < H) {
        const uint8_t* p = src + (size_t)(yb - 3) * pitch + x;
#pragma unroll
        for (int step = 0; step < BT_R + 6; step++, p += pitch) own[step] = loads ? *reinterpret_cast<const uint32_t*>(p) : 0u;
    } else {
#pragma unroll
        for (int step = 0; step < BT_R + 6; step++)
            own[step] = loads ? *reinterpret_cast<const uint32_t*>(src + (unsigned)(reflect101(yb + step - 3, H) * pitch) + x) : 0u;
    }

    uint32_t pk[6][4];
    uint32_t hprev[4] = {0, 0, 0, 0};
#pragma unroll
    for (int step = 0; step < BT_R + 6; step++) {
        const uint32_t W1 = own[step];
        uint32_t W0 = __shfl_up_sync(0xFFFFFFFFu, W1, 1);
        const uint32_t W2 = __shfl_down_sync(0xFFFFFFFFu, W1, 1);
        if (left_edge) W0 = __byte_perm(W1, W2, 0x1234);
        uint32_t h[4];
        h[0] = __dp4a(__byte_perm(W0, W1, 0x4321), WLO, __dp4a(__byte_perm(W1, W2, 0x4321), WHI, 0u));
        h[1] = __dp4a(__byte_perm(W0, W1, 0x5432), WLO, __dp4a(__byte_perm(W1, W2, 0x5432), WHI, 0u));
        h[2] = __dp4a(__byte_perm(W0, W1, 0x6543), WLO, __dp4a(__byte_perm(W1, W2, 0x6543), WHI, 0u));
        h[3] = __dp4a(W1, WLO, __dp4a(W2, WHI, 0u));
        if (step >= 1) {
#pragma unroll
            for (int i = 0; i < 4; i++) pk[(step - 1) % 6][i] = __byte_perm(hprev[i], h[i], 0x5410);
        }
        if (step >= 6) {
            const int yout = yb + step - 6;
            if (yout < H && stores) {
                uint32_t s[4];
#pragma unroll
                for (int i = 0; i < 4; i++) {
                    uint32_t acc = h[i] * 18u + 32768u;
                    acc = __dp2a_lo(pk[(step - 2) % 6][i], 48u | (34u << 8), acc);
                    acc = __dp2a_lo(pk[(step - 4) % 6][i], 48u | (56u << 8), acc);
                    s[i] = __dp2a_lo(pk[(step - 6) % 6][i], 18u | (34u << 8), acc);
                }
                const uint32_t out = __byte_perm(__byte_perm(s[0], s[1], 0x0062), __byte_perm(s[2], s[3], 0x0062), 0x5410);
                *reinterpret_cast<uint32_t*>(dst + (size_t)yout * pitch + x) = out;
            }
        }
#pragma unroll
        for (int i = 0; i < 4; i++) hprev[i] = h[i];
    }
}

int launch_blur(const Geometry& g, const Workspace& ws, int n_images, cudaStream_t s) {
    dim3 grid(g.blur_tiles, n_images);
    blur_kernel<<<grid, 32 * BT_WARPS, 0, s>>>(g, ws.pyr, ws.blur);
    return 1;
}

}
```

### orb_slam2_b200/csrc/k_pyramid.cu

```cuda
#include "borb_internal.h"

namespace borb {

template <int ROWS>
__global__ void __launch_bounds__(256, 6) pyr_resize_kernel(const uint8_t* __restrict__ pyr, uint8_t* __restrict__ pyr_out,
                                                         const int16_t* __restrict__ tabs, LevelGeom src, LevelGeom dst,
                                                         unsigned image_stride) {
    const int img = blockIdx.z;
    const int dyb = (blockIdx.y * 8 + threadIdx.y) * ROWS;
    const int dx0 = (blockIdx.x * 32 + threadIdx.x) * 4;
    const int wpad = (dst.w + 8 + 3) & ~3;
    if (dyb >= dst.h || dx0 >= wpad) return;
    const uint8_t* S = pyr + (size_t)img * image_stride + src.pyr_off;
    uint8_t* D = pyr_out + (size_t)img * image_stride + dst.pyr_off;
    const uint4* xt = reinterpret_cast<const uint4*>(tabs + ((size_t)dst.xwin_off + dx0) * 4);
    const uint2* yt = reinterpret_cast<const uint2*>(tabs + (size_t)dst.ytab_off * 4);
    const uint4 e01 = xt[0], e23 = xt[1];
    const uint32_t wts[4] = {e01.x, e01.z, e23.x, e23.z};
    const uint32_t ctl[4] = {e01.y, e01.w, e23.y, e23.w};
    const int base = (int)(ctl[0] & 0xFFFF);
    uint32_t ra[ROWS][3], rc[ROWS][3];
    uint32_t B0[ROWS], B1[ROWS];
#pragma unroll
    for (int r = 0; r < ROWS; r++) {
        const int dy = min(dyb + r, dst.h - 1);
        const uint2 ye = yt[dy];
        const int sy = (int)(short)(ye.x & 0xFFFF);
        B0[r] = ye.x & 0xFFFF0000u;
        B1[r] = ye.y << 16;
        const int sy0 = min(max(sy, 0), src.h - 1), sy1 = min(max(sy + 1, 0), src.h - 1);
        const uint32_t* R0 = reinterpret_cast<const uint32_t*>(S + (size_t)sy0 * src.pitch + base);
        const uint32_t* R1 = reinterpret_cast<const uint32_t*>(S + (size_t)sy1 * src.pitch + base);
        ra[r][0] = R0[0]; ra[r][1] = R0[1]; ra[r][2] = R0[2];
        rc[r][0] = R1[0]; rc[r][1] = R1[1]; rc[r][2] = R1[2];
    }
#pragma unroll
    for (int r = 0; r < ROWS; r++) {
        if (dyb + r >= dst.h) break;
        uint32_t v[4];
#pragma unroll
        for (int i = 0; i < 4; i++) {
            const uint32_t s1 = ctl[i] >> 16, s2 = ctl[i] >> 24;
            const uint32_t p0 = __byte_perm(__byte_perm(ra[r][0], ra[r][1], s1), ra[r][2], s2);
            const uint32_t p1 = __byte_perm(__byte_perm(rc[r][0], rc[r][1], s1), rc[r][2], s2);
            const uint32_t h0 = __dp2a_lo(wts[i], p0, 0u), h1 = __dp2a_lo(wts[i], p1, 0u);
            v[i] = (__umulhi(B0[r], h0 >> 4) + __umulhi(B1[r], h1 >> 4) + 2) >> 2;
        }
        const uint32_t out = __byte_perm(__byte_perm(v[0], v[1], 0x0040), __byte_perm(v[2], v[3], 0x0040), 0x5410);
        *reinterpret_cast<uint32_t*>(D + (size_t)(dyb + r) * dst.pitch + dx0) = out;
    }
}

__global__ void __launch_bounds__(256) pyr_resize_generic_kernel(const uint8_t* __restrict__ pyr, uint8_t* __restrict__ pyr_out,
                                                                 const int16_t* __restrict__ tabs, LevelGeom src, LevelGeom dst,
                                                                 unsigned image_stride) {
    const int img = blockIdx.z;
    const int dy = blockIdx.y * 8 + threadIdx.y;
    const int dx = blockIdx.x * 32 + threadIdx.x;
    const int wpad = (dst.w + 8 + 3) & ~3;
    if (dy >= dst.h || dx >= wpad) return;
    const uint8_t* S = pyr + (size_t)img * image_stride + src.pyr_off;
    uint8_t* D = pyr_out + (size_t)img * image_stride + dst.pyr_off;
    const short4 xe = reinterpret_cast<const short4*>(tabs)[(size_t)dst.xtab_off + dx];
    const short4 ye = reinterpret_cast<const short4*>(tabs)[(size_t)dst.ytab_off + dy];
    const int sy0 = min(max((int)ye.x, 0), src.h - 1), sy1 = min(max((int)ye.x + 1, 0), src.h - 1);
    const uint8_t* R0 = S + (size_t)sy0 * src.pitch;
    const uint8_t* R1 = S + (size_t)sy1 * src.pitch;
    const int sx = xe.x;
    const int r0 = R0[sx] * xe.y + R0[sx + 1] * xe.z;
    const int r1 = R1[sx] * xe.y + R1[sx + 1] * xe.z;
    D[(size_t)dy * dst.pitch + dx] = (uint8_t)((((ye.y * (r0 >> 4)) >> 16) + ((ye.z * (r1 >> 4)) >> 16) + 2) >> 2);
}

__global__ void __launch_bounds__(256) repack_kernel(const uint8_t* __restrict__ stage, int src_stride, size_t src_image_bytes,
                                                     uint8_t* __restrict__ pyr, LevelGeom l0, unsigned image_stride) {
    const int img = blockIdx.z, y = blockIdx.y;
    const int x0 = (blockIdx.x * 256 + threadIdx.x) * 4;
    if (x0 >= l0.w) return;
    const uint8_t* S = stage + (size_t)img * src_image_bytes + (size_t)y * src_stride + x0;
    uint32_t v = 0;
#pragma unroll
    for (int i = 0; i < 4; i++)
        if (x0 + i < l0.w) v |= (uint32_t)S[i] << (8 * i);
    *reinterpret_cast<uint32_t*>(pyr + (size_t)img * image_stride + l0.pyr_off + (size_t)y * l0.pitch + x0) = v;
}

__global__ void __launch_bounds__(256) repack_color_kernel(const uint8_t* __restrict__ stage, int src_stride, size_t src_image_bytes,
                                                           int channels, int rgb, uint8_t* __restrict__ pyr, LevelGeom l0,
                                                           unsigned image_stride) {
    const int img = blockIdx.z, y = blockIdx.y;
    const int x0 = (blockIdx.x * 256 + threadIdx.x) * 4;
    if (x0 >= l0.w) return;
    const uint8_t* S = stage + (size_t)img * src_image_bytes + (size_t)y * src_stride + (size_t)x0 * channels;
    const int cr = rgb ? 9798 : 3735, cb = rgb ? 3735 : 9798;
    uint32_t v = 0;
#pragma unroll
    for (int i = 0; i < 4; i++)
        if (x0 + i < l0.w) {
            const uint8_t* px = S + i * channels;
            const int yv = (px[0] * cr + px[1] * 19235 + px[2] * cb + 16384) >> 15;
            v |= (uint32_t)yv << (8 * i);
        }
    *reinterpret_cast<uint32_t*>(pyr + (size_t)img * image_stride + l0.pyr_off + (size_t)y * l0.pitch + x0) = v;
}

__global__ void __launch_bounds__(256) repack_remap_kernel(const uint8_t* __restrict__ stage, int src_stride, size_t src_image_bytes,
                                                           int src_w, int src_h, const float* __restrict__ mx0,
                                                           const float* __restrict__ my0, const float* __restrict__ mx1,
                                                           const float* __restrict__ my1, uint8_t* __restrict__ pyr, LevelGeom l0,
                                                           unsigned image_stride) {
    const int img = blockIdx.z, y = blockIdx.y;
    const int x0 = (blockIdx.x * 256 + threadIdx.x) * 4;
    if (x0 >= l0.w) return;
    const bool second = (img & 1) && mx1 != nullptr;
    const float* MX = second ? mx1 : mx0;
    const float* MY = second ? my1 : my0;
    const uint8_t* S = stage + (size_t)img * src_image_bytes;
    uint32_t v = 0;
#pragma unroll
    for (int i = 0; i < 4; i++)
        if (x0 + i < l0.w) {
            const size_t o = (size_t)y * l0.w + x0 + i;
            const int sx = __float2int_rn(__fmul_rn(MX[o], 32.f)), sy = __float2int_rn(__fmul_rn(MY[o], 32.f));
            const int ix = max(-32768, min(32767, sx >> 5)), iy = max(-32768, min(32767, sy >> 5));
            const int fx = sx & 31, fy = sy & 31;
            auto tap = [&](int yy, int xx) -> int {
                return (xx >= 0 && xx < src_w && yy >= 0 && yy < src_h) ? (int)S[(size_t)yy * src_stride + xx] : 0;
            };
            const int w00 = (32 - fx) * (32 - fy) * 32, w01 = fx * (32 - fy) * 32, w10 = (32 - fx) * fy * 32, w11 = fx * fy * 32;
            const int r = (tap(iy, ix) * w00 + tap(iy, ix + 1) * w01 + tap(iy + 1, ix) * w10 + tap(iy + 1, ix + 1) * w11 + 16384) >> 15;
            v |= (uint32_t)r << (8 * i);
        }
    *reinterpret_cast<uint32_t*>(pyr + (size_t)img * image_stride + l0.pyr_off + (size_t)y * l0.pitch + x0) = v;
}

__global__ void __launch_bounds__(256) pad_level0_kernel(uint8_t* __restrict__ pyr, LevelGeom l0, unsigned image_stride) {
    const int y = blockIdx.x * 256 + threadIdx.x, img = blockIdx.y;
    if (y >= l0.h) return;
    uint8_t* row = pyr + (size_t)img * image_stride + l0.pyr_off + (size_t)y * l0.pitch;
#pragma unroll
    for (int k = 0; k < 8; k++) row[l0.w + k] = row[max(l0.w - 2 - k, 0)];
}

int launch_repack(const Geometry& g, const Workspace& ws, const uint8_t* stage, int src_stride, size_t src_image_bytes,
                  int n_images, cudaStream_t s) {
    dim3 grid((g.lv[0].w + 1023) / 1024, g.lv[0].h, n_images);
    repack_kernel<<<grid, 256, 0, s>>>(stage, src_stride, src_image_bytes, ws.pyr, g.lv[0], g.pyr_image_stride);
    return 1;
}

constexpr int PYR_ROWS = 2;

int launch_repack_remap(const Geometry& g, const Workspace& ws, const uint8_t* stage, int src_stride, size_t src_image_bytes, int src_w,
                        int src_h, const float* mx0, const float* my0, const float* mx1, const float* my1, int n_images, cudaStream_t s) {
    dim3 grid((g.lv[0].w + 1023) / 1024, g.lv[0].h, n_images);
    repack_remap_kernel<<<grid, 256, 0, s>>>(stage, src_stride, src_image_bytes, src_w, src_h, mx0, my0, mx1, my1, ws.pyr, g.lv[0],
                                             g.pyr_image_stride);
    return 1;
}

int launch_repack_color(const Geometry& g, const Workspace& ws, const uint8_t* stage, int src_stride, size_t src_image_bytes, int channels,
                        int rgb, int n_images, cudaStream_t s) {
    dim3 grid((g.lv[0].w + 1023) / 1024, g.lv[0].h, n_images);
    repack_color_kernel<<<grid, 256, 0, s>>>(stage, src_stride, src_image_bytes, channels, rgb, ws.pyr, g.lv[0], g.pyr_image_stride);
    return 1;
}

int launch_pyramid(const Geometry& g, const Workspace& ws, int n_images, cudaStream_t s) {
    int launches = 0;
    pad_level0_kernel<<<dim3((g.lv[0].h + 255) / 256, n_images), 256, 0, s>>>(ws.pyr, g.lv[0], g.pyr_image_stride);
    launches++;
    for (int l = 1; l < g.nlevels; l++) {
        const LevelGeom& d = g.lv[l];
        dim3 block(32, 8);
        if (d.x_windowed) {
            dim3 grid((d.w + 8 + 127) / 128, (d.h + 8 * PYR_ROWS - 1) / (8 * PYR_ROWS), n_images);
            pyr_resize_kernel<PYR_ROWS><<<grid, block, 0, s>>>(ws.pyr, ws.pyr, ws.tabs, g.lv[l - 1], d, g.pyr_image_stride);
        } else {
            dim3 grid((d.w + 8 + 3 + 31) / 32, (d.h + 7) / 8, n_images);
            pyr_resize_generic_kernel<<<grid, block, 0, s>>>(ws.pyr, ws.pyr, ws.tabs, g.lv[l - 1], d, g.pyr_image_stride);
        }
        launches++;
    }
    return launches;
}

}
```

Baseline: 36050.

## Fuse pyramid build and Gaussian blur into one persistent dataflow kernel

```diff
diff --git a/include/borb.h b/include/borb.h
--- a/include/borb.h
+++ b/include/borb.h
@@ -335,6 +335,7 @@
 BORB_API borb_status borb_debug_blurred(borb_extractor* e, int image, int level, uint8_t* dst, int* w, int* h);
 BORB_API borb_status borb_debug_set_fast_mode(borb_extractor* e, int mode);
 BORB_API borb_status borb_debug_brief_slots(uint32_t* dst, int cap, int* n_bins);
+BORB_API borb_status borb_debug_pyramid_tasks(const borb_extractor_cfg* cfg, int width, int height, int32_t* dst, int cap, int* n_out);
 BORB_API borb_status borb_debug_set_bow_csa(int mode);
 BORB_API borb_status borb_debug_set_bow_item_target(int target);
 BORB_API borb_status borb_launch_count(const borb_extractor* e, uint64_t* n);
diff --git a/orb_slam2_b200/_lib.py b/orb_slam2_b200/_lib.py
--- a/orb_slam2_b200/_lib.py
+++ b/orb_slam2_b200/_lib.py
@@ -124,6 +124,7 @@
     "borb_debug_set_bow_item_target": (C.c_int, [C.c_int]),
     "borb_debug_set_fast_mode": (C.c_int, [vp, C.c_int]),
     "borb_debug_brief_slots": (C.c_int, [vp, C.c_int, i32p]),
+    "borb_debug_pyramid_tasks": (C.c_int, [C.POINTER(ExtractorCfg), C.c_int, C.c_int, vp, C.c_int, i32p]),
     "borb_launch_count": (C.c_int, [vp, C.POINTER(C.c_uint64)]),
     "borb_stage_times": (C.c_int, [vp, f32p]),
     "borb_set_timing": (C.c_int, [vp, C.c_int]),
diff --git a/orb_slam2_b200/csrc/borb_host.cu b/orb_slam2_b200/csrc/borb_host.cu
--- a/orb_slam2_b200/csrc/borb_host.cu
+++ b/orb_slam2_b200/csrc/borb_host.cu
@@ -136,7 +136,7 @@
     g.min_th = e->cfg.min_th_fast < 0 ? 0 : (e->cfg.min_th_fast > 255 ? 255 : e->cfg.min_th_fast);
     for (int i = 0; i < 16; i++) g.umax[i] = e->umax[i];
     unsigned pyr_off = 0, cand_off = 0;
-    int blk = 0, sel_off = 0, btile = 0;
+    int blk = 0, sel_off = 0, ptask = 0;
     tabs.clear();
     for (int l = 0; l < L; l++) {
         LevelGeom& v = g.lv[l];
@@ -173,8 +173,8 @@
         v.scale = e->scale[l];
         v.inv_scale = e->inv_scale[l];
         v.patch_size = (float)(int)(PATCH * e->scale[l]);
-        g.blur_base[l] = btile;
-        btile += ((v.w + BLUR_TILE_W - 1) / BLUR_TILE_W) * ((v.h + BLUR_TILE_H - 1) / BLUR_TILE_H);
+        g.pt_base[l] = ptask;
+        ptask += (v.h + PYR_BAND_H - 1) / PYR_BAND_H;
         if (l > 0) {
             const int wpad = (v.w + 8 + 3) & ~3;
             v.xtab_off = (unsigned)(tabs.size() / 4);
@@ -191,8 +191,7 @@
             return BORB_ERR_UNSUPPORTED;
         }
     }
-    g.blur_base[L] = btile;
-    g.blur_tiles = btile;
+    g.pt_base[L] = ptask;
     g.fast_blocks = blk;
     g.pyr_image_stride = (unsigned)align_up((int)pyr_off, g.lv[0].pitch);
     g.cand_image_stride = cand_off;
@@ -201,8 +200,47 @@
     return BORB_OK;
 }
 
+std::vector<PyrTask> build_pyr_tasks(const Geometry& g, const std::vector<int16_t>& tabs) {
+    std::vector<PyrTask> out((size_t)g.pt_base[g.nlevels]);
+    auto reflect101 = [](int p, int len) { if (p < 0) p = -p; if (p >= len) p = 2 * len - 2 - p; return std::min(std::max(p, 0), len - 1); };
+    for (int l = 0; l < g.nlevels; l++) {
+        const LevelGeom& v = g.lv[l];
+        const int nb = g.pt_base[l + 1] - g.pt_base[l];
+        for (int b = 0; b < nb; b++) {
+            PyrTask& t = out[(size_t)g.pt_base[l] + b];
+            const int y0 = b * PYR_BAND_H, y1 = std::min(v.h, y0 + PYR_BAND_H);
+            t.y0 = (int16_t)y0; t.y1 = (int16_t)y1;
+            t.src_lo = 0; t.src_hi = -1;
+            if (l > 0) {
+                const int sh = g.lv[l - 1].h;
+                int lo = sh, hi = -1;
+                for (int dy = y0; dy < y1; dy++) {
+                    const int sy = tabs[((size_t)v.ytab_off + dy) * 4];
+                    lo = std::min(lo, std::min(std::max(sy, 0), sh - 1));
+                    hi = std::max(hi, std::min(std::max(sy + 1, 0), sh - 1));
+                }
+                t.src_lo = (int16_t)(lo / PYR_BAND_H); t.src_hi = (int16_t)(hi / PYR_BAND_H);
+            }
+            t.blur_y0 = t.blur_y1 = 0;
+            t.dep_lo = 0; t.dep_hi = -1;
+            if (b > 0 || nb == 1) {
+                const int by0 = b > 0 ? (b - 1) * PYR_BAND_H : 0, by1 = b == nb - 1 ? v.h : y0;
+                t.blur_y0 = (int16_t)by0; t.blur_y1 = (int16_t)by1;
+                int lo = v.h, hi = -1;
+                for (int y = by0 - 3; y < by1 + 3; y++) {
+                    const int r = reflect101(y, v.h);
+                    lo = std::min(lo, r); hi = std::max(hi, r);
+                }
+                t.dep_lo = (int16_t)(lo / PYR_BAND_H);
+                t.dep_hi = (int16_t)std::min(hi / PYR_BAND_H, b - 1);
+            }
+        }
+    }
+    return out;
+}
+
 void free_workspace(Workspace& ws) {
-    cudaFree(ws.pyr); cudaFree(ws.blur); cudaFree(ws.cand); cudaFree(ws.cand_cnt); cudaFree(ws.pnode); cudaFree(ws.sel);
+    cudaFree(ws.pyr); cudaFree(ws.blur); cudaFree(ws.cand); cudaFree(ws.pyr_ticket); cudaFree(ws.pyr_tasks); cudaFree(ws.pyr_flags); cudaFree(ws.pnode); cudaFree(ws.sel);
     cudaFree(ws.sel_cnt); cudaFree(ws.kps); cudaFree(ws.desc); cudaFree(ws.nkp); cudaFree(ws.u_right); cudaFree(ws.depth);
     cudaFree(ws.sad); cudaFree(ws.tabs); cudaFree(ws.brief_slots); cudaFree(ws.pair_idx); cudaFree(ws.st_bins); cudaFree(ws.st_recs); cudaFree(ws.stage);
     free(ws.fast_tmaps); cudaFree(ws.fast_tiles);
@@ -232,7 +270,8 @@
     BORB_CUDA(cudaMalloc(&ws.blur, n * g.pyr_image_stride + 256));
     BORB_CUDA(cudaMalloc(&ws.cand, n * g.cand_image_stride * sizeof(uint32_t)));
     BORB_CUDA(cudaMalloc(&ws.pnode, n * g.cand_image_stride * sizeof(int)));
-    BORB_CUDA(cudaMalloc(&ws.cand_cnt, n * g.nlevels * sizeof(int)));
+    BORB_CUDA(cudaMalloc(&ws.pyr_ticket, (1 + n * g.nlevels) * sizeof(int)));
+    ws.cand_cnt = ws.pyr_ticket + 1;
     BORB_CUDA(cudaMalloc(&ws.sel, n * g.sel_image_stride * sizeof(uint32_t)));
     BORB_CUDA(cudaMalloc(&ws.sel_cnt, n * g.nlevels * sizeof(int)));
     BORB_CUDA(cudaMalloc(&ws.kps, n * g.sel_image_stride * sizeof(borb_keypoint)));
@@ -246,6 +285,12 @@
     BORB_CUDA(cudaMalloc(&ws.st_recs, n * (size_t)stereo_rec_stride(g) * stereo_rec_bytes()));
     BORB_CUDA(cudaMalloc(&ws.tabs, (tabs.size() + 4) * sizeof(int16_t)));
     BORB_CUDA(cudaMemcpy(ws.tabs, tabs.data(), tabs.size() * sizeof(int16_t), cudaMemcpyHostToDevice));
+    const std::vector<PyrTask> ptasks = build_pyr_tasks(g, tabs);
+    BORB_CUDA(cudaMalloc(&ws.pyr_tasks, ptasks.size() * sizeof(PyrTask)));
+    BORB_CUDA(cudaMemcpy(ws.pyr_tasks, ptasks.data(), ptasks.size() * sizeof(PyrTask), cudaMemcpyHostToDevice));
+    BORB_CUDA(cudaMalloc(&ws.pyr_flags, n * ptasks.size() * sizeof(unsigned)));
+    BORB_CUDA(cudaMemset(ws.pyr_flags, 0, n * ptasks.size() * sizeof(unsigned)));
+    if ((ws.pyr_ctas = pyr_blur_resident_ctas()) < 1) { set_error("pyr_blur_kernel: occupancy query failed"); return BORB_ERR_CUDA; }
     const std::vector<uint32_t>& slots = brief_slot_table();
     BORB_CUDA(cudaMalloc(&ws.brief_slots, slots.size() * sizeof(uint32_t)));
     BORB_CUDA(cudaMemcpy(ws.brief_slots, slots.data(), slots.size() * sizeof(uint32_t), cudaMemcpyHostToDevice));
@@ -303,7 +348,7 @@
     const Geometry& g = e->geom;
     Workspace& ws = e->ws;
     cudaStream_t s = e->stream;
-    BORB_CUDA(cudaMemsetAsync(ws.cand_cnt, 0, (size_t)n * g.nlevels * sizeof(int), s));
+    BORB_CUDA(cudaMemsetAsync(ws.pyr_ticket, 0, (1 + (size_t)n * g.nlevels) * sizeof(int), s));
     mark(e, 1);
     e->launches += launch_pyramid(g, ws, n, s);
     mark(e, 2);
@@ -311,7 +356,6 @@
     mark(e, 3);
     e->launches += launch_quadtree(g, ws, n, s);
     mark(e, 4);
-    e->launches += launch_blur(g, ws, n, s);
     mark(e, 5);
     e->launches += launch_describe(g, ws, n, s);
     mark(e, 6);
@@ -790,6 +834,31 @@
     return BORB_OK;
 }
 
+borb_status borb_debug_pyramid_tasks(const borb_extractor_cfg* cfg, int width, int height, int32_t* dst, int cap, int* n_out) {
+    if (!cfg || !n_out) { set_error("null argument"); return BORB_ERR_INVALID_ARG; }
+    if (cfg->n_levels < 1 || cfg->n_levels > BORB_MAX_LEVELS || cfg->n_features < 1 || !(cfg->scale_factor > 1.0f)) {
+        set_error("bad extractor cfg"); return BORB_ERR_INVALID_ARG;
+    }
+    if (width < 1 || height < 1 || width > BORB_MAX_DIM || height > BORB_MAX_DIM) { set_error("image size out of range"); return BORB_ERR_UNSUPPORTED; }
+    borb_extractor tmp;
+    tmp.cfg = *cfg;
+    init_tables(&tmp);
+    std::vector<int16_t> tabs;
+    borb_status st = build_geometry(&tmp, width, height, tabs);
+    if (st != BORB_OK) return st;
+    const Geometry& g = tmp.geom;
+    const std::vector<PyrTask> t = build_pyr_tasks(g, tabs);
+    *n_out = (int)t.size();
+    for (int l = 0, k = 0; l < g.nlevels; l++)
+        for (int b = 0; b < g.pt_base[l + 1] - g.pt_base[l]; b++, k++) {
+            if (!dst || k >= cap) continue;
+            const PyrTask& x = t[k];
+            const int32_t row[10] = {l, b, x.y0, x.y1, x.src_lo, x.src_hi, x.blur_y0, x.blur_y1, x.dep_lo, x.dep_hi};
+            std::memcpy(dst + (size_t)k * 10, row, sizeof(row));
+        }
+    return BORB_OK;
+}
+
 borb_status borb_launch_count(const borb_extractor* e, uint64_t* n) {
     if (!e || !n) return BORB_ERR_INVALID_ARG;
     *n = e->launches;
diff --git a/orb_slam2_b200/csrc/borb_internal.h b/orb_slam2_b200/csrc/borb_internal.h
--- a/orb_slam2_b200/csrc/borb_internal.h
+++ b/orb_slam2_b200/csrc/borb_internal.h
@@ -17,7 +17,7 @@
 constexpr int TH_HIGH = 100;
 constexpr int TH_LOW = 50;
 constexpr int BLUR_TILE_W = 120;
-constexpr int BLUR_TILE_H = 64;
+constexpr int PYR_BAND_H = 32;
 constexpr int FAST_TILE_W = 124;
 constexpr int FAST_H_BAND = 64;
 
@@ -56,6 +56,13 @@
     int x_windowed;
 };
 
+struct alignas(16) PyrTask {
+    int16_t y0, y1;
+    int16_t src_lo, src_hi;
+    int16_t blur_y0, blur_y1;
+    int16_t dep_lo, dep_hi;
+};
+
 struct Geometry {
     int nlevels;
     int w, h;
@@ -65,8 +72,7 @@
     unsigned pyr_image_stride;
     unsigned cand_image_stride;
     int sel_image_stride;
-    int blur_tiles;
-    int blur_base[BORB_MAX_LEVELS + 1];
+    int pt_base[BORB_MAX_LEVELS + 1];
     int umax[16];
     LevelGeom lv[BORB_MAX_LEVELS];
 };
@@ -76,6 +82,7 @@
     uint8_t* pyr = nullptr;
     uint8_t* blur = nullptr;
     uint32_t* cand = nullptr;
+    int* pyr_ticket = nullptr;
     int* cand_cnt = nullptr;
     int* pnode = nullptr;
     uint32_t* sel = nullptr;
@@ -87,6 +94,10 @@
     float* depth = nullptr;
     int* sad = nullptr;
     int16_t* tabs = nullptr;
+    PyrTask* pyr_tasks = nullptr;
+    unsigned* pyr_flags = nullptr;
+    unsigned pyr_epoch = 0;
+    int pyr_ctas = 0;
     uint32_t* brief_slots = nullptr;
     int* pair_idx = nullptr;
     int* st_bins = nullptr;
@@ -118,10 +129,10 @@
                         int rgb, int n_images, cudaStream_t s);
 int launch_repack(const Geometry& g, const Workspace& ws, const uint8_t* stage, int src_stride, size_t src_image_bytes,
                   int n_images, cudaStream_t s);
-int launch_pyramid(const Geometry& g, const Workspace& ws, int n_images, cudaStream_t s);
+int launch_pyramid(const Geometry& g, Workspace& ws, int n_images, cudaStream_t s);
+int pyr_blur_resident_ctas();
 int launch_fast(const Geometry& g, const Workspace& ws, int n_images, cudaStream_t s);
 int launch_quadtree(const Geometry& g, const Workspace& ws, int n_images, cudaStream_t s);
-int launch_blur(const Geometry& g, const Workspace& ws, int n_images, cudaStream_t s);
 int launch_describe(const Geometry& g, const Workspace& ws, int n_images, cudaStream_t s);
 
 struct StereoView {
diff --git a/orb_slam2_b200/csrc/k_blur.cu b/orb_slam2_b200/csrc/k_blur.cu
--- a/orb_slam2_b200/csrc/k_blur.cu
+++ /dev/null
@@ -1,92 +0,0 @@
-#include "borb_internal.h"
-
-namespace borb {
-
-namespace {
-constexpr int BT_R = 16;
-constexpr int BT_WARPS = BLUR_TILE_H / BT_R;
-
-__device__ __forceinline__ int reflect101(int p, int len) {
-    if (p < 0) p = -p;
-    if (p >= len) p = 2 * len - 2 - p;
-    return min(max(p, 0), len - 1);
-}
-}
-
-__global__ void __launch_bounds__(32 * BT_WARPS) blur_kernel(const __grid_constant__ Geometry g, const uint8_t* __restrict__ pyr,
-                                                             uint8_t* __restrict__ blur) {
-    const int img = blockIdx.y;
-    int l = 0;
-    while (l + 1 < g.nlevels && (int)blockIdx.x >= g.blur_base[l + 1]) l++;
-    const LevelGeom& L = g.lv[l];
-    const int local = blockIdx.x - g.blur_base[l];
-    const int tilesX = (L.w + BLUR_TILE_W - 1) / BLUR_TILE_W;
-    const int ty = local / tilesX, tx = local - ty * tilesX;
-    const int lane = threadIdx.x & 31, wrp = threadIdx.x >> 5;
-    const int x = tx * BLUR_TILE_W + 4 * (lane - 1);
-    const int yb = ty * BLUR_TILE_H + wrp * BT_R;
-    if (yb >= L.h) return;
-    const uint8_t* src = pyr + (size_t)img * g.pyr_image_stride + L.pyr_off;
-    uint8_t* dst = blur + (size_t)img * g.pyr_image_stride + L.pyr_off;
-    const int W = L.w, H = L.h, pitch = L.pitch;
-    const bool left_edge = (x == 0);
-    const bool loads = x >= 0 && x < pitch;
-    const bool stores = lane >= 1 && lane <= 30 && x < W;
-    const unsigned WLO = 18u | (34u << 8) | (48u << 16) | (56u << 24);
-    const unsigned WHI = 48u | (34u << 8) | (18u << 16);
-
-    uint32_t own[BT_R + 6];
-    if (yb >= 3 && yb + BT_R + 2 < H) {
-        const uint8_t* p = src + (size_t)(yb - 3) * pitch + x;
-#pragma unroll
-        for (int step = 0; step < BT_R + 6; step++, p += pitch) own[step] = loads ? *reinterpret_cast<const uint32_t*>(p) : 0u;
-    } else {
-#pragma unroll
-        for (int step = 0; step < BT_R + 6; step++)
-            own[step] = loads ? *reinterpret_cast<const uint32_t*>(src + (unsigned)(reflect101(yb + step - 3, H) * pitch) + x) : 0u;
-    }
-
-    uint32_t pk[6][4];
-    uint32_t hprev[4] = {0, 0, 0, 0};
-#pragma unroll
-    for (int step = 0; step < BT_R + 6; step++) {
-        const uint32_t W1 = own[step];
-        uint32_t W0 = __shfl_up_sync(0xFFFFFFFFu, W1, 1);
-        const uint32_t W2 = __shfl_down_sync(0xFFFFFFFFu, W1, 1);
-        if (left_edge) W0 = __byte_perm(W1, W2, 0x1234);
-        uint32_t h[4];
-        h[0] = __dp4a(__byte_perm(W0, W1, 0x4321), WLO, __dp4a(__byte_perm(W1, W2, 0x4321), WHI, 0u));
-        h[1] = __dp4a(__byte_perm(W0, W1, 0x5432), WLO, __dp4a(__byte_perm(W1, W2, 0x5432), WHI, 0u));
-        h[2] = __dp4a(__byte_perm(W0, W1, 0x6543), WLO, __dp4a(__byte_perm(W1, W2, 0x6543), WHI, 0u));
-        h[3] = __dp4a(W1, WLO, __dp4a(W2, WHI, 0u));
-        if (step >= 1) {
-#pragma unroll
-            for (int i = 0; i < 4; i++) pk[(step - 1) % 6][i] = __byte_perm(hprev[i], h[i], 0x5410);
-        }
-        if (step >= 6) {
-            const int yout = yb + step - 6;
-            if (yout < H && stores) {
-                uint32_t s[4];
-#pragma unroll
-                for (int i = 0; i < 4; i++) {
-                    uint32_t acc = h[i] * 18u + 32768u;
-                    acc = __dp2a_lo(pk[(step - 2) % 6][i], 48u | (34u << 8), acc);
-                    acc = __dp2a_lo(pk[(step - 4) % 6][i], 48u | (56u << 8), acc);
-                    s[i] = __dp2a_lo(pk[(step - 6) % 6][i], 18u | (34u << 8), acc);
-                }
-                const uint32_t out = __byte_perm(__byte_perm(s[0], s[1], 0x0062), __byte_perm(s[2], s[3], 0x0062), 0x5410);
-                *reinterpret_cast<uint32_t*>(dst + (size_t)yout * pitch + x) = out;
-            }
-        }
-#pragma unroll
-        for (int i = 0; i < 4; i++) hprev[i] = h[i];
-    }
-}
-
-int launch_blur(const Geometry& g, const Workspace& ws, int n_images, cudaStream_t s) {
-    dim3 grid(g.blur_tiles, n_images);
-    blur_kernel<<<grid, 32 * BT_WARPS, 0, s>>>(g, ws.pyr, ws.blur);
-    return 1;
-}
-
-}
diff --git a/orb_slam2_b200/csrc/k_pyramid.cu b/orb_slam2_b200/csrc/k_pyramid.cu
--- a/orb_slam2_b200/csrc/k_pyramid.cu
+++ b/orb_slam2_b200/csrc/k_pyramid.cu
@@ -2,65 +2,94 @@
 
 namespace borb {
 
+namespace {
+
+constexpr int PYR_THREADS = 256;
+constexpr int PYR_WARPS = PYR_THREADS / 32;
+constexpr int PYR_ROWS = 4;
+constexpr int BT_R = 16;
+static_assert(PYR_BAND_H % BT_R == 0, "a blur item must not straddle two bands");
+static_assert(PYR_BAND_H % PYR_ROWS == 0, "a resize item must not straddle two bands");
+static_assert(PYR_THREADS == PYR_BAND_H * 8, "level-0 padding: one thread per (row, padding byte) of a band");
+
+__device__ __forceinline__ int reflect101(int p, int len) {
+    if (p < 0) p = -p;
+    if (p >= len) p = 2 * len - 2 - p;
+    return min(max(p, 0), len - 1);
+}
+
+__device__ __forceinline__ unsigned ld_acquire(const unsigned* p) {
+    unsigned v;
+    asm volatile("ld.acquire.gpu.global.u32 %0, [%1];" : "=r"(v) : "l"(p) : "memory");
+    return v;
+}
+__device__ __forceinline__ void st_release(unsigned* p, unsigned v) {
+    asm volatile("st.release.gpu.global.u32 [%0], %1;" ::"l"(p), "r"(v) : "memory");
+}
+
+__device__ __forceinline__ void wait_bands(const unsigned* f, int lo, int hi, unsigned epoch) {
+    for (int i = lo + (int)threadIdx.x; i <= hi; i += PYR_THREADS)
+        while (ld_acquire(f + i) != epoch) __nanosleep(64);
+    __syncthreads();
+}
+
 template <int ROWS>
-__global__ void __launch_bounds__(256, 6) pyr_resize_kernel(const uint8_t* __restrict__ pyr, uint8_t* __restrict__ pyr_out,
-                                                         const int16_t* __restrict__ tabs, LevelGeom src, LevelGeom dst,
-                                                         unsigned image_stride) {
-    const int img = blockIdx.z;
-    const int dyb = (blockIdx.y * 8 + threadIdx.y) * ROWS;
-    const int dx0 = (blockIdx.x * 32 + threadIdx.x) * 4;
+__device__ __forceinline__ void resize_window_rows(const uint8_t* S, uint8_t* D, const int16_t* __restrict__ tabs, const LevelGeom& src,
+                                                   const LevelGeom& dst, int dyb, int yend, int lane) {
     const int wpad = (dst.w + 8 + 3) & ~3;
-    if (dyb >= dst.h || dx0 >= wpad) return;
-    const uint8_t* S = pyr + (size_t)img * image_stride + src.pyr_off;
-    uint8_t* D = pyr_out + (size_t)img * image_stride + dst.pyr_off;
-    const uint4* xt = reinterpret_cast<const uint4*>(tabs + ((size_t)dst.xwin_off + dx0) * 4);
     const uint2* yt = reinterpret_cast<const uint2*>(tabs + (size_t)dst.ytab_off * 4);
-    const uint4 e01 = xt[0], e23 = xt[1];
-    const uint32_t wts[4] = {e01.x, e01.z, e23.x, e23.z};
-    const uint32_t ctl[4] = {e01.y, e01.w, e23.y, e23.w};
-    const int base = (int)(ctl[0] & 0xFFFF);
-    uint32_t ra[ROWS][3], rc[ROWS][3];
+    const uint8_t* R0[ROWS];
+    const uint8_t* R1[ROWS];
     uint32_t B0[ROWS], B1[ROWS];
 #pragma unroll
     for (int r = 0; r < ROWS; r++) {
-        const int dy = min(dyb + r, dst.h - 1);
+        const int dy = min(dyb + r, yend - 1);
         const uint2 ye = yt[dy];
         const int sy = (int)(short)(ye.x & 0xFFFF);
         B0[r] = ye.x & 0xFFFF0000u;
         B1[r] = ye.y << 16;
         const int sy0 = min(max(sy, 0), src.h - 1), sy1 = min(max(sy + 1, 0), src.h - 1);
-        const uint32_t* R0 = reinterpret_cast<const uint32_t*>(S + (size_t)sy0 * src.pitch + base);
-        const uint32_t* R1 = reinterpret_cast<const uint32_t*>(S + (size_t)sy1 * src.pitch + base);
-        ra[r][0] = R0[0]; ra[r][1] = R0[1]; ra[r][2] = R0[2];
-        rc[r][0] = R1[0]; rc[r][1] = R1[1]; rc[r][2] = R1[2];
-    }
-#pragma unroll
-    for (int r = 0; r < ROWS; r++) {
-        if (dyb + r >= dst.h) break;
-        uint32_t v[4];
-#pragma unroll
-        for (int i = 0; i < 4; i++) {
-            const uint32_t s1 = ctl[i] >> 16, s2 = ctl[i] >> 24;
-            const uint32_t p0 = __byte_perm(__byte_perm(ra[r][0], ra[r][1], s1), ra[r][2], s2);
-            const uint32_t p1 = __byte_perm(__byte_perm(rc[r][0], rc[r][1], s1), rc[r][2], s2);
-            const uint32_t h0 = __dp2a_lo(wts[i], p0, 0u), h1 = __dp2a_lo(wts[i], p1, 0u);
-            v[i] = (__umulhi(B0[r], h0 >> 4) + __umulhi(B1[r], h1 >> 4) + 2) >> 2;
-        }
-        const uint32_t out = __byte_perm(__byte_perm(v[0], v[1], 0x0040), __byte_perm(v[2], v[3], 0x0040), 0x5410);
-        *reinterpret_cast<uint32_t*>(D + (size_t)(dyb + r) * dst.pitch + dx0) = out;
-    }
-}
-
-__global__ void __launch_bounds__(256) pyr_resize_generic_kernel(const uint8_t* __restrict__ pyr, uint8_t* __restrict__ pyr_out,
-                                                                 const int16_t* __restrict__ tabs, LevelGeom src, LevelGeom dst,
-                                                                 unsigned image_stride) {
-    const int img = blockIdx.z;
-    const int dy = blockIdx.y * 8 + threadIdx.y;
-    const int dx = blockIdx.x * 32 + threadIdx.x;
-    const int wpad = (dst.w + 8 + 3) & ~3;
-    if (dy >= dst.h || dx >= wpad) return;
-    const uint8_t* S = pyr + (size_t)img * image_stride + src.pyr_off;
-    uint8_t* D = pyr_out + (size_t)img * image_stride + dst.pyr_off;
+        R0[r] = S + (size_t)sy0 * src.pitch;
+        R1[r] = S + (size_t)sy1 * src.pitch;
+    }
+    const uint4* xt = reinterpret_cast<const uint4*>(tabs + (size_t)dst.xwin_off * 4);
+    int dx0 = lane * 4;
+    uint4 n01 = make_uint4(0, 0, 0, 0), n23 = n01;
+    if (dx0 < wpad) { n01 = xt[dx0 / 2]; n23 = xt[dx0 / 2 + 1]; }
+    for (; dx0 < wpad; dx0 += 128) {
+        const uint4 e01 = n01, e23 = n23;
+        if (dx0 + 128 < wpad) { n01 = xt[(dx0 + 128) / 2]; n23 = xt[(dx0 + 128) / 2 + 1]; }
+        const uint32_t wts[4] = {e01.x, e01.z, e23.x, e23.z};
+        const uint32_t ctl[4] = {e01.y, e01.w, e23.y, e23.w};
+        const int base = (int)(ctl[0] & 0xFFFF);
+        uint32_t ra[ROWS][3], rc[ROWS][3];
+#pragma unroll
+        for (int r = 0; r < ROWS; r++) {
+            const uint32_t* W0 = reinterpret_cast<const uint32_t*>(R0[r] + base);
+            const uint32_t* W1 = reinterpret_cast<const uint32_t*>(R1[r] + base);
+            ra[r][0] = W0[0]; ra[r][1] = W0[1]; ra[r][2] = W0[2];
+            rc[r][0] = W1[0]; rc[r][1] = W1[1]; rc[r][2] = W1[2];
+        }
+#pragma unroll
+        for (int r = 0; r < ROWS; r++) {
+            if (dyb + r >= yend) break;
+            uint32_t v[4];
+#pragma unroll
+            for (int i = 0; i < 4; i++) {
+                const uint32_t s1 = ctl[i] >> 16, s2 = ctl[i] >> 24;
+                const uint32_t p0 = __byte_perm(__byte_perm(ra[r][0], ra[r][1], s1), ra[r][2], s2);
+                const uint32_t p1 = __byte_perm(__byte_perm(rc[r][0], rc[r][1], s1), rc[r][2], s2);
+                const uint32_t h0 = __dp2a_lo(wts[i], p0, 0u), h1 = __dp2a_lo(wts[i], p1, 0u);
+                v[i] = (__umulhi(B0[r], h0 >> 4) + __umulhi(B1[r], h1 >> 4) + 2) >> 2;
+            }
+            const uint32_t out = __byte_perm(__byte_perm(v[0], v[1], 0x0040), __byte_perm(v[2], v[3], 0x0040), 0x5410);
+            *reinterpret_cast<uint32_t*>(D + (size_t)(dyb + r) * dst.pitch + dx0) = out;
+        }
+    }
+}
+
+__device__ __forceinline__ void resize_generic_px(const uint8_t* S, uint8_t* D, const int16_t* __restrict__ tabs, const LevelGeom& src,
+                                                  const LevelGeom& dst, int dy, int dx) {
     const short4 xe = reinterpret_cast<const short4*>(tabs)[(size_t)dst.xtab_off + dx];
     const short4 ye = reinterpret_cast<const short4*>(tabs)[(size_t)dst.ytab_off + dy];
     const int sy0 = min(max((int)ye.x, 0), src.h - 1), sy1 = min(max((int)ye.x + 1, 0), src.h - 1);
@@ -70,6 +99,63 @@
     const int r0 = R0[sx] * xe.y + R0[sx + 1] * xe.z;
     const int r1 = R1[sx] * xe.y + R1[sx + 1] * xe.z;
     D[(size_t)dy * dst.pitch + dx] = (uint8_t)((((ye.y * (r0 >> 4)) >> 16) + ((ye.z * (r1 >> 4)) >> 16) + 2) >> 2);
+}
+
+__device__ __forceinline__ void blur_strip(const uint8_t* src, uint8_t* dst, int W, int H, int pitch, int x, int yb, int yend, int lane) {
+    const bool left_edge = (x == 0);
+    const bool loads = x >= 0 && x < pitch;
+    const bool stores = lane >= 1 && lane <= 30 && x < W;
+    const unsigned WLO = 18u | (34u << 8) | (48u << 16) | (56u << 24);
+    const unsigned WHI = 48u | (34u << 8) | (18u << 16);
+
+    uint32_t own[BT_R + 6];
+    if (yb >= 3 && yb + BT_R + 2 < H) {
+        const uint8_t* p = src + (size_t)(yb - 3) * pitch + x;
+#pragma unroll
+        for (int step = 0; step < BT_R + 6; step++, p += pitch) own[step] = loads ? *reinterpret_cast<const uint32_t*>(p) : 0u;
+    } else {
+#pragma unroll
+        for (int step = 0; step < BT_R + 6; step++)
+            own[step] = loads ? *reinterpret_cast<const uint32_t*>(src + (unsigned)(reflect101(yb + step - 3, H) * pitch) + x) : 0u;
+    }
+
+    uint32_t pk[6][4];
+    uint32_t hprev[4] = {0, 0, 0, 0};
+#pragma unroll
+    for (int step = 0; step < BT_R + 6; step++) {
+        const uint32_t W1 = own[step];
+        uint32_t W0 = __shfl_up_sync(0xFFFFFFFFu, W1, 1);
+        const uint32_t W2 = __shfl_down_sync(0xFFFFFFFFu, W1, 1);
+        if (left_edge) W0 = __byte_perm(W1, W2, 0x1234);
+        uint32_t h[4];
+        h[0] = __dp4a(__byte_perm(W0, W1, 0x4321), WLO, __dp4a(__byte_perm(W1, W2, 0x4321), WHI, 0u));
+        h[1] = __dp4a(__byte_perm(W0, W1, 0x5432), WLO, __dp4a(__byte_perm(W1, W2, 0x5432), WHI, 0u));
+        h[2] = __dp4a(__byte_perm(W0, W1, 0x6543), WLO, __dp4a(__byte_perm(W1, W2, 0x6543), WHI, 0u));
+        h[3] = __dp4a(W1, WLO, __dp4a(W2, WHI, 0u));
+        if (step >= 1) {
+#pragma unroll
+            for (int i = 0; i < 4; i++) pk[(step - 1) % 6][i] = __byte_perm(hprev[i], h[i], 0x5410);
+        }
+        if (step >= 6) {
+            const int yout = yb + step - 6;
+            if (yout < yend && stores) {
+                uint32_t s[4];
+#pragma unroll
+                for (int i = 0; i < 4; i++) {
+                    uint32_t acc = h[i] * 18u + 32768u;
+                    acc = __dp2a_lo(pk[(step - 2) % 6][i], 48u | (34u << 8), acc);
+                    acc = __dp2a_lo(pk[(step - 4) % 6][i], 48u | (56u << 8), acc);
+                    s[i] = __dp2a_lo(pk[(step - 6) % 6][i], 18u | (34u << 8), acc);
+                }
+                const uint32_t out = __byte_perm(__byte_perm(s[0], s[1], 0x0062), __byte_perm(s[2], s[3], 0x0062), 0x5410);
+                *reinterpret_cast<uint32_t*>(dst + (size_t)yout * pitch + x) = out;
+            }
+        }
+#pragma unroll
+        for (int i = 0; i < 4; i++) hprev[i] = h[i];
+    }
+}
+
 }
 
 __global__ void __launch_bounds__(256) repack_kernel(const uint8_t* __restrict__ stage, int src_stride, size_t src_image_bytes,
@@ -134,12 +220,80 @@
     *reinterpret_cast<uint32_t*>(pyr + (size_t)img * image_stride + l0.pyr_off + (size_t)y * l0.pitch + x0) = v;
 }
 
-__global__ void __launch_bounds__(256) pad_level0_kernel(uint8_t* __restrict__ pyr, LevelGeom l0, unsigned image_stride) {
-    const int y = blockIdx.x * 256 + threadIdx.x, img = blockIdx.y;
-    if (y >= l0.h) return;
-    uint8_t* row = pyr + (size_t)img * image_stride + l0.pyr_off + (size_t)y * l0.pitch;
-#pragma unroll
-    for (int k = 0; k < 8; k++) row[l0.w + k] = row[max(l0.w - 2 - k, 0)];
+__global__ void __launch_bounds__(PYR_THREADS, 3) pyr_blur_kernel(const __grid_constant__ Geometry g, uint8_t* pyr, uint8_t* blur,
+                                                               const int16_t* __restrict__ tabs, const PyrTask* __restrict__ tasks,
+                                                               int* ticket, unsigned* flags, int n_images, unsigned epoch) {
+    __shared__ int s_ticket;
+    const int tid = threadIdx.x, lane = tid & 31, wrp = tid >> 5;
+    const int per_image = g.pt_base[g.nlevels];
+    const int total = n_images * per_image;
+    for (;;) {
+        if (tid == 0) s_ticket = atomicAdd(ticket, 1);
+        __syncthreads();
+        const int t = s_ticket;
+        if (t >= total) return;
+        int l = 0;
+        while (l + 1 < g.nlevels && t >= n_images * g.pt_base[l + 1]) l++;
+        const int nb = g.pt_base[l + 1] - g.pt_base[l];
+        const int rem = t - n_images * g.pt_base[l];
+        const int img = rem / nb, b = rem - img * nb;
+        const PyrTask tk = tasks[g.pt_base[l] + b];
+        unsigned* fl = flags + (size_t)img * per_image;
+        const LevelGeom& L = g.lv[l];
+        uint8_t* P = pyr + (size_t)img * g.pyr_image_stride;
+        uint8_t* D = P + L.pyr_off;
+
+        if (l == 0) {
+            const int y = tk.y0 + (tid >> 3), k = tid & 7;
+            if (y < tk.y1) D[(size_t)y * L.pitch + L.w + k] = D[(size_t)y * L.pitch + max(L.w - 2 - k, 0)];
+        } else {
+            const LevelGeom& Sg = g.lv[l - 1];
+            wait_bands(fl + g.pt_base[l - 1], tk.src_lo, tk.src_hi, epoch);
+            const uint8_t* S = P + Sg.pyr_off;
+            const int wpad = (L.w + 8 + 3) & ~3;
+            if (L.x_windowed) {
+                for (int dyb = tk.y0 + wrp * PYR_ROWS; dyb < tk.y1; dyb += PYR_WARPS * PYR_ROWS)
+                    resize_window_rows<PYR_ROWS>(S, D, tabs, Sg, L, dyb, tk.y1, lane);
+            } else {
+                for (int dy = tk.y0 + wrp; dy < tk.y1; dy += PYR_WARPS)
+                    for (int dx = lane; dx < wpad; dx += 32) resize_generic_px(S, D, tabs, Sg, L, dy, dx);
+            }
+        }
+        __syncthreads();
+        if (tid == 0) st_release(fl + g.pt_base[l] + b, epoch);
+
+        if (tk.blur_y0 < tk.blur_y1) {
+            wait_bands(fl + g.pt_base[l], tk.dep_lo, tk.dep_hi, epoch);
+            uint8_t* B = blur + (size_t)img * g.pyr_image_stride + L.pyr_off;
+            const int strips = (L.w + BLUR_TILE_W - 1) / BLUR_TILE_W;
+            const int items = strips * ((tk.blur_y1 - tk.blur_y0 + BT_R - 1) / BT_R);
+            for (int it = wrp; it < items; it += PYR_WARPS) {
+                const int c = it / strips, sx = it - c * strips;
+                const int yb = tk.blur_y0 + c * BT_R;
+                blur_strip(D, B, L.w, L.h, L.pitch, sx * BLUR_TILE_W + 4 * (lane - 1), yb, min(yb + BT_R, (int)tk.blur_y1), lane);
+            }
+        }
+    }
+}
+
+int pyr_blur_resident_ctas() {
+    int dev = 0, sms = 0, per_sm = 0;
+    if (cudaGetDevice(&dev) != cudaSuccess || cudaDeviceGetAttribute(&sms, cudaDevAttrMultiProcessorCount, dev) != cudaSuccess ||
+        cudaOccupancyMaxActiveBlocksPerMultiprocessor(&per_sm, pyr_blur_kernel, PYR_THREADS, 0) != cudaSuccess)
+        return 0;
+    return sms * per_sm;
+}
+
+int launch_pyramid(const Geometry& g, Workspace& ws, int n_images, cudaStream_t s) {
+    if (++ws.pyr_epoch == 0) {
+        cudaMemsetAsync(ws.pyr_flags, 0, (size_t)ws.max_images * g.pt_base[g.nlevels] * sizeof(unsigned), s);
+        ws.pyr_epoch = 1;
+    }
+    const int tasks = n_images * g.pt_base[g.nlevels];
+    const int grid = tasks < ws.pyr_ctas ? tasks : ws.pyr_ctas;
+    pyr_blur_kernel<<<grid, PYR_THREADS, 0, s>>>(g, ws.pyr, ws.blur, ws.tabs, ws.pyr_tasks, ws.pyr_ticket, ws.pyr_flags, n_images,
+                                                 ws.pyr_epoch);
+    return 1;
 }
 
 int launch_repack(const Geometry& g, const Workspace& ws, const uint8_t* stage, int src_stride, size_t src_image_bytes,
@@ -148,8 +302,6 @@
     repack_kernel<<<grid, 256, 0, s>>>(stage, src_stride, src_image_bytes, ws.pyr, g.lv[0], g.pyr_image_stride);
     return 1;
 }
-
-constexpr int PYR_ROWS = 2;
 
 int launch_repack_remap(const Geometry& g, const Workspace& ws, const uint8_t* stage, int src_stride, size_t src_image_bytes, int src_w,
                         int src_h, const float* mx0, const float* my0, const float* mx1, const float* my1, int n_images, cudaStream_t s) {
@@ -166,23 +318,4 @@
     return 1;
 }
 
-int launch_pyramid(const Geometry& g, const Workspace& ws, int n_images, cudaStream_t s) {
-    int launches = 0;
-    pad_level0_kernel<<<dim3((g.lv[0].h + 255) / 256, n_images), 256, 0, s>>>(ws.pyr, g.lv[0], g.pyr_image_stride);
-    launches++;
-    for (int l = 1; l < g.nlevels; l++) {
-        const LevelGeom& d = g.lv[l];
-        dim3 block(32, 8);
-        if (d.x_windowed) {
-            dim3 grid((d.w + 8 + 127) / 128, (d.h + 8 * PYR_ROWS - 1) / (8 * PYR_ROWS), n_images);
-            pyr_resize_kernel<PYR_ROWS><<<grid, block, 0, s>>>(ws.pyr, ws.pyr, ws.tabs, g.lv[l - 1], d, g.pyr_image_stride);
-        } else {
-            dim3 grid((d.w + 8 + 3 + 31) / 32, (d.h + 7) / 8, n_images);
-            pyr_resize_generic_kernel<<<grid, block, 0, s>>>(ws.pyr, ws.pyr, ws.tabs, g.lv[l - 1], d, g.pyr_image_stride);
-        }
-        launches++;
-    }
-    return launches;
-}
-
-}
+}
```

New measurement: 36410 (median of 6 runs). 1.01x the previous value.
